# thuml/iVideoGPT

Hardware: AMD Instinct MI355X
Metric: predicted frames/sec (encode+GPT rollout+decode), 64x64x16f (higher is better)
Workload: dtype bf16; 1 GPU; ivideogpt-oxe-64-act-free (BASELINE config 2): synthetic 64x64 bf16 clips, 64 trajectories per GPU, 2 context + 14 predicted frames, top-k 100 sampling, seeded random weights; global_batch=64, frames=16, resolution=64, lanes=4

## Files before the change

include/ivg.h:

```cpp
#ifndef IVG_H_
#define IVG_H_

#include <stddef.h>
#include <stdint.h>

#ifdef __cplusplus
extern "C" {
#endif

typedef struct ivg_engine ivg_engine;
typedef struct ivg_cache ivg_cache;
typedef void* ivg_stream;

enum ivg_dtype { IVG_F32 = 0, IVG_BF16 = 1, IVG_F32X3 = 2 };

enum ivg_status {
  IVG_OK = 0,
  IVG_ERR_INVALID = -1,
  IVG_ERR_MISSING = -2,
  IVG_ERR_HIP = -3,
  IVG_ERR_CAPACITY = -4
};

typedef struct {
// ... 92 lines not shown
                        void* hidden_out, int allow_reuse, int* reused_out, ivg_stream stream);
int ivg_reward_linear(ivg_engine* e, const void* hidden, int rows, float* out, ivg_stream stream);

int ivg_logits(ivg_engine* e, const int64_t* ids, int B, int L, const float* actions, int act_T, int ctx, float* logits_out,
               ivg_stream stream);

int ivg_eval_forward(ivg_engine* e, const int64_t* ids, const int64_t* labels, int B, int L, const float* actions, int act_T, int ctx,
                     float* token_nll_out, float* loss_rows_out, void* hidden_out, ivg_stream stream);
int ivg_action_recon_sqerr(ivg_engine* e, const void* hidden, const float* actions, int B, int L, int act_T, int ctx, int prelude, float* out,
                           ivg_stream stream);

int ivg_ingest_frames(const uint8_t* frames, int T, int H, int W, int center_crop, void* clip_out, int out_dtype, int resolution,
                      ivg_stream stream);

size_t ivg_frame_metrics_ws_bytes(int n_samples, int T, int H, int W);
int ivg_frame_metrics(const void* gt, int gt_dtype, int B, int T_gt, int gt_t0, const float* pred, int n_samples, int T_pr, int pr_t0, int T, int H,
                      int W, float* rows_out, void* ws, size_t ws_bytes, ivg_stream stream);

typedef struct ivg_lpips ivg_lpips;
int ivg_lpips_create(const ivg_tensor* weights, int n_weights, int device, ivg_lpips** out);
void ivg_lpips_destroy(ivg_lpips* p);
size_t ivg_lpips_ws_bytes(int max_images_per_chunk, int H, int W);
int ivg_lpips_rows(ivg_lpips* p, const void* gt, int gt_dtype, int B, int T_gt, int gt_t0, const float* pred, int n_samples, int T_pr, int pr_t0, int T,
                   int H, int W, float* frames_out, float* rows_out, void* ws, size_t ws_bytes, ivg_stream stream);

enum ivg_kernel_class { IVG_K_IGEMM_BF16 = 0, IVG_K_IGEMM_F32 = 1, IVG_K_CONV3X3_BF16 = 2, IVG_K_CONV3X3_F32 = 3, IVG_K_DECODE_ATTN = 4,
                        IVG_K_DECODE_GEMM = 5,
                        IVG_K_COUNT = 6 };
typedef struct {
  int64_t launches;
  double total_ms;
  double total_flops;
  double total_bytes;
} ivg_profile_stats;
int ivg_profile_enable(ivg_engine* e, int kernel_class, int enable);
int ivg_profile_read(ivg_engine* e, int kernel_class, ivg_profile_stats* out);
int ivg_profile_attn_fit(ivg_engine* e, double* fixed_us, double* gbps);
int ivg_profile_gemm_kinds(ivg_engine* e, double* mean_us, int64_t* launches);

typedef struct {
  const void* X; const void* W; void* Y; const void* R; const float* bias;
  int32_t Nimg, Hin, Win, Cin, ldx, Hout, Wout, KH, KW, stride, pad, ups, N, ldw;
  int64_t c_img, c_pix, c_ch, c_grp_stride;
  int32_t c_grp, flags;
  float alpha;
  int32_t nb0, nb1, nb2;
  int64_t sa[3], sw[3], sy[3];
} ivg_igemm_args;
int ivg_op_igemm(const ivg_igemm_args* a, int dtype, ivg_stream stream);
int ivg_op_conv_gn(const ivg_igemm_args* a, int dtype, void* gn_part, int groups, const float* gamma, const float* beta, void* gn_out, float eps,
                   int silu, ivg_stream stream);
int ivg_op_gn_conv(const ivg_igemm_args* a, int dtype, int groups, const float* gamma, const float* beta, float eps, void* ws, ivg_stream stream);
int ivg_op_conv_x3(const ivg_igemm_args* a, const void* w_x3, int groups, const float* gamma, const float* beta, float eps, void* ws,
                   ivg_stream stream);
int ivg_op_conv_subpixel(const ivg_igemm_args* a, int dtype, const void* w_sub, const void* w_x3, const void* w_sub_x3, void* gn_part, int groups,
                         ivg_stream stream);
int ivg_op_conv3x3(const ivg_igemm_args* a, int dtype, const float* gamma, const float* beta, int in_groups, float eps, void* ws,
                   const void* in_part, int in_chunks, void* gn_part, int groups, const void* w_x3, const void* w_sub, const void* w_sub_x3,
                   ivg_stream stream);
#define IVG_CONV3X3_PLAN_INTS 15
int ivg_op_conv3x3_plan(const ivg_igemm_args* a, int dtype, int gn_in, int gn_groups, const void* w_x3, const void* w_sub,
                        const void* w_sub_x3, int32_t* out);
int ivg_op_xattn(const void* q, const void* Kp, const void* VpT, void* out, int M, int F, int P, int kv, int C, int nh, int dtype, ivg_stream stream);
int ivg_op_skinny(const void* X, const void* W, void* Y, int M, int N, int K, int ldx, int ldw, int ldy, int flags, int dtype,
                  ivg_stream stream);
int ivg_op_skinny_policy(const void* X, const void* W, void* Y, int M, int N, int K, int ldx, int ldw, int ldy, int flags, int dtype, int lds_kb,
                         int w_shared, ivg_stream stream);
#define IVG_SKINNY_PLAN_INTS 11
int ivg_op_skinny_plan(int M, int N, int K, int ldx, int ldw, int ldy, int flags, int dtype, int lds_kb, const void* X, const void* W,
                       const void* Y, int32_t* out);
int ivg_op_groupnorm(const void* X, void* Y, void* ws , const float* gamma, const float* beta,
                     const float* pos, int N, int P, int C, int groups, float eps, int silu, int dtype, ivg_stream stream);
int ivg_op_softmax(const float* S, void* P, int64_t rows, int Lq, int Lk, int lds, int ldp, int causal, int dtype,
                   ivg_stream stream);
int ivg_op_vq_argmin(const float* z, const float* codebook, float* ee_ws , int64_t* out, int R, int n_e,
                     ivg_stream stream);
int ivg_op_add_rmsnorm(void* x, const float* w, void* out, int M, int H, float eps, int dtype, ivg_stream stream);
int ivg_op_conv_in(const void* video, int video_dtype, const float* w, const float* bias, void* Y, int dtype, int N, int per,
                   int T_total, int t0, int H, int W, int C0, ivg_stream stream);
int ivg_op_shared_decode_attn(const void* qkv, void* kc, void* vc, void* out, const float* cos_t, const float* sin_t, int B, int heads, int hd, int Lmax,
                              int pos, int P, int G, int row0, int dtype, ivg_stream stream);
int ivg_op_prefill_attn(void* qkv, void* kc, void* vc, void* vt, void* out, const float* cos_t, const float* sin_t, int B, int L, int heads, int hd,
                        int Lmax, int dtype, ivg_stream stream);
int ivg_op_kv24_pack(const float* k32, const float* v32, void* kc, void* vc, int BH, int L, int Lmax, ivg_stream stream);
int ivg_op_decode_attn24(const float* qkv, void* kc, void* vc, float* out, const float* cos_t, const float* sin_t, int B, int heads, int Lmax, int pos,
                         int P, int G, int row0, ivg_stream stream);
int ivg_op_kv8_pack(const void* k16, const void* v16, void* kc, void* vc, int BH, int L, int Lmax, float k_scale, float v_scale, ivg_stream stream);
int ivg_op_decode_attn8(const void* qkv, void* kc, void* vc, void* out, const float* cos_t, const float* sin_t, int B, int heads, int Lmax, int pos,
                        int P, int G, int row0, float k_scale, float v_scale, ivg_stream stream);
int ivg_op_kv8_pack_heads(const void* k16, const void* v16, void* kc, void* vc, int B, int heads, int L, int Lmax, const float* k_scales,
                          const float* v_scales, ivg_stream stream);
int ivg_op_decode_attn8_heads(const void* qkv, void* kc, void* vc, void* out, const float* cos_t, const float* sin_t, int B, int heads, int Lmax, int pos,
                              int P, int G, int row0, const float* k_scales, const float* v_scales, ivg_stream stream);
int ivg_op_kv_absmax(const void* k16, const void* v16, int B, int heads, int L, int Lmax, uint32_t* out, ivg_stream stream);
int ivg_op_sample(const float* logits, int B, int V, int top_k, float temperature, const float* uniforms, int64_t* out, ivg_stream stream);
int ivg_op_sample_top_p(const float* logits, int B, int V, int top_k, float temperature, float top_p, const float* uniforms, int64_t* out,
                        ivg_stream stream);
int ivg_op_lpips_features(ivg_lpips* p, const void* images, int dtype, int n, int H, int W, float* const* taps_out, void* ws, size_t ws_bytes,
                          ivg_stream stream);
int ivg_op_lpips_head(const float* f0, const float* f1, const float* lin, int n0, int n1, int P, int C, float* out, void* ws, size_t ws_bytes,
                      ivg_stream stream);
int ivg_op_lpips_conv_in(const void* images, int dtype, const float* w, const float* bias, float* Y, int n, int H, int W, ivg_stream stream);
int ivg_op_maxpool2(const float* X, float* Y, int N, int H, int W, int C, ivg_stream stream);
int64_t ivg_debug_counter(const char* name);

#ifdef __cplusplus
}
#endif
#endif
```

ivideogpt_amd/_lib.py:

```python
import ctypes as C
import os

_HERE = os.path.dirname(os.path.abspath(__file__))
LIB_PATH = os.path.join(_HERE, "lib", "libivg.so")

IVG_F32, IVG_BF16, IVG_F32X3 = 0, 1, 2
IVG_K_IGEMM_BF16, IVG_K_IGEMM_F32, IVG_K_CONV3X3_BF16, IVG_K_CONV3X3_F32, IVG_K_DECODE_ATTN, IVG_K_DECODE_GEMM = 0, 1, 2, 3, 4, 5
IG_BIAS_N, IG_BIAS_M, IG_RESIDUAL, IG_SILU, IG_GLU, IG_OUT_F32 = 1, 2, 4, 8, 16, 32
IG_RELU = 256
IVG_KV_NATIVE, IVG_KV_FP8_E4M3 = 0, 1


class IvgTensor(C.Structure):
    _fields_ = [("name", C.c_char_p), ("data", C.c_void_p), ("dtype", C.c_int32), ("ndim", C.c_int32),
                ("shape", C.c_int64 * 4)]


class IvgConfig(C.Structure):
    _fields_ = [
        ("n_levels", C.c_int32), ("block_out_channels", C.c_int32 * 8), ("layers_per_block", C.c_int32),
        ("latent_channels", C.c_int32), ("vq_embed_dim", C.c_int32), ("num_vq_embeddings", C.c_int32),
        ("num_dyn_embeddings", C.c_int32), ("norm_num_groups", C.c_int32), ("mid_block_add_attention", C.c_int32),
        ("context_length", C.c_int32), ("max_att_resolution", C.c_int32), ("resolution", C.c_int32),
        ("patch_size", C.c_int32),
# ... 30 lines not shown
    "ivg_create": (C.c_int, [C.POINTER(IvgConfig), C.POINTER(IvgTensor), C.c_int, C.c_int, C.POINTER(C.c_void_p)]),
    "ivg_destroy": (None, [C.c_void_p]),
    "ivg_reload_switches": (None, []),
    "ivg_set_temperature": (C.c_int, [C.c_void_p, C.c_float]),
    "ivg_set_top_p": (C.c_int, [C.c_void_p, C.c_float]),
    "ivg_set_decode_lds_kb": (C.c_int, [C.c_void_p, C.c_int]),
    "ivg_set_kv_format": (C.c_int, [C.c_void_p, C.c_int, C.c_float, C.c_float]),
    "ivg_set_kv_scales": (C.c_int, [C.c_void_p, C.c_void_p]),
    "ivg_get_kv_scales": (C.c_int, [C.c_void_p, C.c_void_p]),
    "ivg_kv_calibrate": (C.c_int, [C.c_void_p, C.c_void_p, C.c_int64, C.c_int, C.c_int, C.c_void_p, C.c_int, C.c_int, C.c_void_p]),
    "ivg_kv_calibration_reset": (C.c_int, [C.c_void_p]),
    "ivg_kv_calibration_finish": (C.c_int, [C.c_void_p, C.c_int, C.c_void_p, C.c_void_p]),
    "ivg_set_context_length": (C.c_int, [C.c_void_p, C.c_int]),
    "ivg_tokenize": (C.c_int, [C.c_void_p, C.c_void_p, C.c_int, C.c_int, C.c_int, C.c_void_p, C.c_void_p, C.c_void_p]),
    "ivg_encode_context": (C.c_int, [C.c_void_p, C.c_void_p, C.c_int, C.c_int, C.c_int, C.c_void_p, C.c_int64, C.c_void_p]),
    "ivg_detokenize": (C.c_int, [C.c_void_p, C.c_void_p, C.c_int, C.c_int, C.c_void_p, C.c_void_p, C.c_int, C.c_void_p]),
    "ivg_detokenize_shared": (C.c_int, [C.c_void_p, C.c_void_p, C.c_int, C.c_int, C.c_int, C.c_void_p, C.c_int, C.c_void_p]),
    "ivg_detokenize_to": (C.c_int, [C.c_void_p, C.c_void_p, C.c_int, C.c_int, C.c_void_p, C.c_int, C.c_void_p, C.c_int, C.c_void_p]),
    "ivg_set_output_clamp": (C.c_int, [C.c_void_p, C.c_int]),
    "ivg_cache_create": (C.c_int, [C.c_void_p, C.c_int, C.POINTER(C.c_void_p)]),
    "ivg_cache_destroy": (None, [C.c_void_p, C.c_void_p]),
    "ivg_generate": (C.c_int, [C.c_void_p, C.c_void_p, C.c_int64, C.c_int, C.c_int, C.c_int, C.c_void_p, C.c_int, C.c_int,
                               C.c_void_p, C.c_int, C.c_void_p, C.c_void_p, C.c_void_p]),
    "ivg_generate_shared": (C.c_int, [C.c_void_p, C.c_void_p, C.c_int64, C.c_int, C.c_int, C.c_int, C.c_int, C.c_void_p, C.c_int, C.c_int,
                                      C.c_void_p, C.c_int, C.c_int, C.c_void_p, C.c_void_p, C.c_void_p]),
    "ivg_generate_forced_sdf": (C.c_int, [C.c_void_p, C.c_void_p, C.c_int64, C.c_int, C.c_int, C.c_int, C.c_int, C.c_void_p, C.c_int, C.c_void_p,
                                         C.c_void_p]),
    "ivg_generate_continue": (C.c_int, [C.c_void_p, C.c_void_p, C.c_int64, C.c_int, C.c_int, C.c_int, C.c_void_p, C.c_int, C.c_int,
                                        C.c_void_p, C.c_int, C.c_void_p, C.c_void_p, C.c_void_p]),
    "ivg_embed_tokens": (C.c_int, [C.c_void_p, C.c_void_p, C.c_int64, C.c_int, C.c_int, C.c_void_p, C.c_void_p]),
    "ivg_action_linear": (C.c_int, [C.c_void_p, C.c_void_p, C.c_int, C.c_void_p, C.c_void_p]),
    "ivg_generate_embeds": (C.c_int, [C.c_void_p, C.c_void_p, C.c_int, C.c_int, C.c_int, C.c_void_p, C.c_int, C.c_void_p, C.c_void_p,
                                      C.c_int, C.POINTER(C.c_int), C.c_void_p]),
    "ivg_reward_linear": (C.c_int, [C.c_void_p, C.c_void_p, C.c_int, C.c_void_p, C.c_void_p]),
    "ivg_logits": (C.c_int, [C.c_void_p, C.c_void_p, C.c_int, C.c_int, C.c_void_p, C.c_int, C.c_int, C.c_void_p, C.c_void_p]),
    "ivg_eval_forward": (C.c_int, [C.c_void_p, C.c_void_p, C.c_void_p, C.c_int, C.c_int, C.c_void_p, C.c_int, C.c_int, C.c_void_p,
                                   C.c_void_p, C.c_void_p, C.c_void_p]),
    "ivg_action_recon_sqerr": (C.c_int, [C.c_void_p, C.c_void_p, C.c_void_p, C.c_int, C.c_int, C.c_int, C.c_int, C.c_int, C.c_void_p,
                                         C.c_void_p]),
    "ivg_ingest_frames": (C.c_int, [C.c_void_p, C.c_int, C.c_int, C.c_int, C.c_int, C.c_void_p, C.c_int, C.c_int, C.c_void_p]),
    "ivg_frame_metrics_ws_bytes": (C.c_size_t, [C.c_int, C.c_int, C.c_int, C.c_int]),
    "ivg_frame_metrics": (C.c_int, [C.c_void_p, C.c_int, C.c_int, C.c_int, C.c_int, C.c_void_p, C.c_int, C.c_int, C.c_int, C.c_int, C.c_int,
                                    C.c_int, C.c_void_p, C.c_void_p, C.c_size_t, C.c_void_p]),
    "ivg_lpips_create": (C.c_int, [C.POINTER(IvgTensor), C.c_int, C.c_int, C.POINTER(C.c_void_p)]),
    "ivg_lpips_destroy": (None, [C.c_void_p]),
    "ivg_lpips_ws_bytes": (C.c_size_t, [C.c_int, C.c_int, C.c_int]),
    "ivg_lpips_rows": (C.c_int, [C.c_void_p, C.c_void_p] + [C.c_int] * 4 + [C.c_void_p] + [C.c_int] * 6 + [C.c_void_p] * 3 + [C.c_size_t, C.c_void_p]),
    "ivg_op_lpips_features": (C.c_int, [C.c_void_p, C.c_void_p] + [C.c_int] * 4 + [C.POINTER(C.c_void_p), C.c_void_p, C.c_size_t, C.c_void_p]),
    "ivg_op_lpips_head": (C.c_int, [C.c_void_p] * 3 + [C.c_int] * 4 + [C.c_void_p, C.c_void_p, C.c_size_t, C.c_void_p]),
    "ivg_op_lpips_conv_in": (C.c_int, [C.c_void_p, C.c_int, C.c_void_p, C.c_void_p, C.c_void_p] + [C.c_int] * 3 + [C.c_void_p]),
    "ivg_op_maxpool2": (C.c_int, [C.c_void_p, C.c_void_p] + [C.c_int] * 4 + [C.c_void_p]),
    "ivg_profile_enable": (C.c_int, [C.c_void_p, C.c_int, C.c_int]),
    "ivg_profile_read": (C.c_int, [C.c_void_p, C.c_int, C.POINTER(IvgProfileStats)]),
    "ivg_profile_attn_fit": (C.c_int, [C.c_void_p, C.POINTER(C.c_double), C.POINTER(C.c_double)]),
    "ivg_profile_gemm_kinds": (C.c_int, [C.c_void_p, C.POINTER(C.c_double), C.POINTER(C.c_int64)]),
    "ivg_op_igemm": (C.c_int, [C.POINTER(IvgIgemmArgs), C.c_int, C.c_void_p]),
    "ivg_op_conv_gn": (C.c_int, [C.POINTER(IvgIgemmArgs), C.c_int, C.c_void_p, C.c_int, C.c_void_p, C.c_void_p, C.c_void_p, C.c_float, C.c_int,
                                 C.c_void_p]),
    "ivg_op_gn_conv": (C.c_int, [C.POINTER(IvgIgemmArgs), C.c_int, C.c_int, C.c_void_p, C.c_void_p, C.c_float, C.c_void_p, C.c_void_p]),
    "ivg_op_conv_x3": (C.c_int, [C.POINTER(IvgIgemmArgs), C.c_void_p, C.c_int, C.c_void_p, C.c_void_p, C.c_float, C.c_void_p, C.c_void_p]),
    "ivg_op_conv3x3": (C.c_int, [C.POINTER(IvgIgemmArgs), C.c_int, C.c_void_p, C.c_void_p, C.c_int, C.c_float, C.c_void_p, C.c_void_p, C.c_int,
                                 C.c_void_p, C.c_int, C.c_void_p, C.c_void_p, C.c_void_p, C.c_void_p]),
    "ivg_op_conv3x3_plan": (C.c_int, [C.POINTER(IvgIgemmArgs), C.c_int, C.c_int, C.c_int, C.c_void_p, C.c_void_p, C.c_void_p,
                                      C.POINTER(C.c_int32)]),
    "ivg_op_xattn": (C.c_int, [C.c_void_p] * 4 + [C.c_int] * 7 + [C.c_void_p]),
    "ivg_op_conv_subpixel": (C.c_int, [C.c_void_p, C.c_int, C.c_void_p, C.c_void_p, C.c_void_p, C.c_void_p, C.c_int, C.c_void_p]),
    "ivg_op_shared_decode_attn": (C.c_int, [C.c_void_p] * 6 + [C.c_int] * 9 + [C.c_void_p]),
    "ivg_op_prefill_attn": (C.c_int, [C.c_void_p] * 7 + [C.c_int] * 6 + [C.c_void_p]),
    "ivg_op_kv24_pack": (C.c_int, [C.c_void_p] * 4 + [C.c_int] * 3 + [C.c_void_p]),
    "ivg_op_decode_attn24": (C.c_int, [C.c_void_p] * 6 + [C.c_int] * 7 + [C.c_void_p]),
    "ivg_op_kv8_pack": (C.c_int, [C.c_void_p] * 4 + [C.c_int] * 3 + [C.c_float, C.c_float, C.c_void_p]),
    "ivg_op_decode_attn8": (C.c_int, [C.c_void_p] * 6 + [C.c_int] * 7 + [C.c_float, C.c_float, C.c_void_p]),
    "ivg_op_kv8_pack_heads": (C.c_int, [C.c_void_p] * 4 + [C.c_int] * 4 + [C.c_void_p] * 3),
    "ivg_op_decode_attn8_heads": (C.c_int, [C.c_void_p] * 6 + [C.c_int] * 7 + [C.c_void_p] * 3),
    "ivg_op_kv_absmax": (C.c_int, [C.c_void_p] * 2 + [C.c_int] * 4 + [C.c_void_p] * 2),
    "ivg_op_skinny": (C.c_int, [C.c_void_p, C.c_void_p, C.c_void_p] + [C.c_int] * 8 + [C.c_void_p]),
    "ivg_op_skinny_policy": (C.c_int, [C.c_void_p, C.c_void_p, C.c_void_p] + [C.c_int] * 10 + [C.c_void_p]),
    "ivg_op_skinny_plan": (C.c_int, [C.c_int] * 9 + [C.c_void_p] * 3 + [C.POINTER(C.c_int32)]),
    "ivg_op_groupnorm": (C.c_int, [C.c_void_p] * 6 + [C.c_int] * 4 + [C.c_float, C.c_int, C.c_int, C.c_void_p]),
    "ivg_op_softmax": (C.c_int, [C.c_void_p, C.c_void_p, C.c_int64] + [C.c_int] * 6 + [C.c_void_p]),
    "ivg_op_vq_argmin": (C.c_int, [C.c_void_p] * 4 + [C.c_int, C.c_int, C.c_void_p]),
    "ivg_op_add_rmsnorm": (C.c_int, [C.c_void_p, C.c_void_p, C.c_void_p, C.c_int, C.c_int, C.c_float, C.c_int, C.c_void_p]),
    "ivg_op_conv_in": (C.c_int, [C.c_void_p, C.c_int, C.c_void_p, C.c_void_p, C.c_void_p] + [C.c_int] * 8 + [C.c_void_p]),
    "ivg_op_sample": (C.c_int, [C.c_void_p, C.c_int, C.c_int, C.c_int, C.c_float, C.c_void_p, C.c_void_p, C.c_void_p]),
    "ivg_op_sample_top_p": (C.c_int, [C.c_void_p, C.c_int, C.c_int, C.c_int, C.c_float, C.c_float, C.c_void_p, C.c_void_p, C.c_void_p]),
    "ivg_debug_counter": (C.c_int64, [C.c_char_p]),
}

_lib = None


def load():
    global _lib
    if _lib is not None:
        return _lib
    if not os.path.exists(LIB_PATH):
        raise RuntimeError(
            f"{LIB_PATH} is missing: the HIP engine has not been built (make -C ivideogpt_amd/csrc). "
            "ivideogpt_amd has no CPU / PyTorch fallback path.")
    lib = C.CDLL(LIB_PATH)
    for name, (res, args) in EXPORTS.items():
        fn = getattr(lib, name)
        fn.restype, fn.argtypes = res, args
    _lib = lib
    return lib


def reload_switches():
    load().ivg_reload_switches()


def last_error(handle=None):
    msg = load().ivg_last_error(handle)
    return msg.decode() if msg else ""


class IvgError(RuntimeError):
    pass


def check(rc, handle=None, what=""):
    if rc != 0:
        msg = f"{what}: libivg error {rc}: {last_error(handle)}"
        if rc == -1:
            raise AssertionError(msg)
        raise IvgError(msg)
```

ivideogpt_amd/csrc/api.cpp:

```cpp
#include <cstdlib>
#include <cstring>

#include <cstdio>
#include "engine_impl.h"
#include "switches.h"

using namespace ivg;

static thread_local std::string g_create_err;

namespace ivg {

size_t dtype_size(DType d) { return d == BF16 ? 2 : 4; }

struct Lookup {
  ivg_engine* e;
  bool ok = true;
  const ivg_tensor* find(const std::string& name, int dtype, int64_t numel) {
    auto it = e->wmap.find(name);
    if (it == e->wmap.end()) { if (ok) e->err = "missing weight tensor '" + name + "'"; ok = false; return nullptr; }
    const ivg_tensor& t = it->second;
    int64_t n = 1;
    for (int i = 0; i < t.ndim; ++i) n *= t.shape[i];
    if (t.dtype != dtype || n != numel) {
// ... 585 lines not shown
                        ivg_stream stream) {
  if (!e) return IVG_ERR_INVALID;
  const bool sized = n_groups > 0 && group_size > 0;
  const int B = sized ? n_groups * group_size : 1;
  IVG_TRY(check_generate(e, GEN_SHARED, sized ? nullptr : "generate_shared: n_groups and group_size must be positive", B, L0, n_new, actions, act_T, ctx));
  GenerateReq q; q.prompt = prompts; q.prompt_stride = prompt_stride; q.B = B; q.L0 = L0; q.n_new = n_new; q.actions = actions; q.act_T = act_T; q.ctx = ctx;
  q.uniforms = uniforms; q.top_k = top_k; q.ids_out = ids_out; q.reward_out = reward_out; q.force_sdf = force_sdf != 0;
  q.group = group_size;
  return plan_then_run(e, (hipStream_t)stream, [&](Run& r) { return r.generate(q); });
}

int ivg_generate_forced_sdf(ivg_engine* e, const int64_t* prompt, int64_t prompt_stride, int B, int L0, int n_new, int ctx, const float* uniforms,
                            int top_k, int64_t* ids_out, ivg_stream stream) {
  if (!e) return IVG_ERR_INVALID;
  IVG_TRY(check_generate(e, GEN_PLAIN, nullptr, B, L0, n_new, nullptr, 0, ctx));
  GenerateReq q; q.prompt = prompt; q.prompt_stride = prompt_stride; q.B = B; q.L0 = L0; q.n_new = n_new; q.ctx = ctx;
  q.uniforms = uniforms; q.top_k = top_k; q.ids_out = ids_out; q.force_sdf = true;
  return plan_then_run(e, (hipStream_t)stream, [&](Run& r) { return r.generate(q); });
}

int ivg_generate_continue(ivg_engine* e, const int64_t* prompt, int64_t prompt_stride, int B, int L0, int n_new, const float* actions,
                          int act_T, int ctx, const float* uniforms, int top_k, int64_t* ids_out, float* reward_out, ivg_stream stream) {
  if (!e) return IVG_ERR_INVALID;
  const bool act_ok = actions && e->cfg.action_dim > 0 && e->act_w;
  IVG_TRY(check_generate(e, GEN_CONTINUE, act_ok ? nullptr : "generate_continue: action-conditioned models only", B, L0, n_new, actions, act_T, ctx));
  if (!e->kvc.holds(B, L0 - 1))
    return e->fail(IVG_ERR_INVALID, "generate_continue: the KV cache holds " + std::to_string(e->kvc.len) + " positions of " + std::to_string(e->kvc.B) +
                                        " trajectories, the call needs " + std::to_string(L0 - 1) + " of " + std::to_string(B));
  {
    bool same = false;
    IVG_TRY(kv_prefix_matches_ids(e, prompt, prompt_stride, B, L0, actions, act_T, ctx, (hipStream_t)stream, &same));
    if (!same) return e->fail(IVG_ERR_INVALID, "generate_continue: the KV cache was built from a different prefix (tokens or actions differ)");
  }
  GenerateReq q; q.prompt = prompt; q.prompt_stride = prompt_stride; q.B = B; q.L0 = L0; q.n_new = n_new; q.actions = actions; q.act_T = act_T; q.ctx = ctx;
  q.uniforms = uniforms; q.top_k = top_k; q.ids_out = ids_out; q.reward_out = reward_out; q.reuse_kv = true;
  return plan_then_run(e, (hipStream_t)stream, [&](Run& r) { return r.generate(q); });
}

int ivg_generate_embeds(ivg_engine* e, const void* embeds, int B, int L0, int n_new, const float* uniforms, int top_k, int64_t* new_ids_out,
                        void* hidden_out, int allow_reuse, int* reused_out, ivg_stream stream) {
  if (!e) return IVG_ERR_INVALID;
  if (reused_out) *reused_out = 0;
  IVG_TRY(check_generate(e, GEN_EMBEDS, embeds && new_ids_out ? nullptr : "generate_embeds: null argument", B, L0, n_new, nullptr, 0, 1));
  bool reuse = false;
  if (allow_reuse && L0 >= 2) IVG_TRY(kv_prefix_matches_embeds(e, embeds, B, L0, (hipStream_t)stream, &reuse));
  if (reused_out) *reused_out = reuse ? 1 : 0;
  GenerateReq q; q.B = B; q.L0 = L0; q.n_new = n_new; q.uniforms = uniforms; q.top_k = top_k;
  q.reuse_kv = reuse; q.embeds = embeds; q.new_ids_out = new_ids_out; q.hidden_out = hidden_out;
  return plan_then_run(e, (hipStream_t)stream, [&](Run& r) { return r.generate(q); });
}

int ivg_embed_tokens(ivg_engine* e, const int64_t* ids, int64_t ids_stride, int B, int L, void* out, ivg_stream stream) {
  if (!e) return IVG_ERR_INVALID;
  if (e->cfg.num_layers <= 0 || !e->embed) return e->fail(IVG_ERR_INVALID, "embed_tokens: engine was created without a transformer");
  if (B <= 0 || L <= 0) return IVG_OK;
  if (launch_embed(ids, ids_stride, e->embed, out, e->llm_dt, B, L, e->cfg.hidden_size, e->cfg.vocab_size, (hipStream_t)stream))
    return e->fail(IVG_ERR_HIP, "embed_tokens: launch failed");
  return IVG_OK;
}

int ivg_action_linear(ivg_engine* e, const float* actions, int rows, void* out, ivg_stream stream) {
  if (!e) return IVG_ERR_INVALID;
  if (e->cfg.action_dim <= 0 || !e->act_w) return e->fail(IVG_ERR_INVALID, "action_linear: the model is action-free");
  if (launch_action_embed(actions, e->act_w, e->act_b, out, e->llm_dt, rows, e->cfg.action_dim, e->cfg.hidden_size, (hipStream_t)stream))
    return e->fail(IVG_ERR_HIP, "action_linear: launch failed");
  return IVG_OK;
}

int ivg_reward_linear(ivg_engine* e, const void* hidden, int rows, float* out, ivg_stream stream) {
  if (!e) return IVG_ERR_INVALID;
  if (!e->rew_w_raw || !e->rew_b) return e->fail(IVG_ERR_MISSING, "reward_linear: the model has no reward head");
  if (launch_rowdot(hidden, e->rew_w_raw, e->rew_b, out, rows, e->cfg.hidden_size, -1.0f, e->llm_dt, (hipStream_t)stream))
    return e->fail(IVG_ERR_HIP, "reward_linear: launch failed");
  return IVG_OK;
}

int ivg_logits(ivg_engine* e, const int64_t* ids, int B, int L, const float* actions, int act_T, int ctx, float* logits_out, ivg_stream stream) {
  if (!e) return IVG_ERR_INVALID;
  if (e->cfg.num_layers <= 0) return e->fail(IVG_ERR_INVALID, "logits: engine was created without a transformer");
  if (B <= 0 || B > e->kvc.chunk || L > e->Lmax) return e->fail(IVG_ERR_CAPACITY, "logits: batch or length exceeds capacity");
  if (actions && (e->cfg.action_dim <= 0 || !e->act_w)) return e->fail(IVG_ERR_INVALID, "logits: actions given but the model is action-free");
  return plan_then_run(e, (hipStream_t)stream, [&](Run& r) {
    PrefillReq q; q.ids = ids; q.ids_stride = L; q.B = B; q.L = L; q.act_T = act_T; q.ctx = ctx; q.all_slots = true; q.logits_all = logits_out;
    IVG_TRY(embed_actions(r, actions, B * act_T, &q.act_emb));
    return r.prefill(q);
  });
}

int ivg_eval_forward(ivg_engine* e, const int64_t* ids, const int64_t* labels, int B, int L, const float* actions, int act_T, int ctx,
                     float* token_nll_out, float* loss_rows_out, void* hidden_out, ivg_stream stream) {
  if (!e) return IVG_ERR_INVALID;
  if (e->cfg.num_layers <= 0) return e->fail(IVG_ERR_INVALID, "eval_forward: engine was created without a transformer");
  if (!ids || !labels || !token_nll_out || !loss_rows_out) return e->fail(IVG_ERR_INVALID, "eval_forward: null argument");
  if (B <= 0 || B > e->kvc.chunk || L < 2 || L > e->Lmax) return e->fail(IVG_ERR_CAPACITY, "eval_forward: batch or length exceeds capacity");
  if (actions && (e->cfg.action_dim <= 0 || !e->act_w)) return e->fail(IVG_ERR_INVALID, "eval_forward: actions given but the model is action-free");
  return plan_then_run(e, (hipStream_t)stream, [&](Run& r) {
    PrefillReq q; q.ids = ids; q.ids_stride = L; q.B = B; q.L = L; q.act_T = act_T; q.ctx = ctx; q.all_slots = true;
    q.hidden_all = hidden_out; q.labels = labels; q.token_nll = token_nll_out;
    IVG_TRY(embed_actions(r, actions, B * act_T, &q.act_emb));
    IVG_TRY(r.prefill(q));
    if (!r.planning && launch_ce_reduce(token_nll_out, labels, B, L, e->cfg.vocab_size, loss_rows_out, r.st)) return e->fail(IVG_ERR_HIP, "ce_reduce launch failed");
    return 0;
  });
}

int ivg_action_recon_sqerr(ivg_engine* e, const void* hidden, const float* actions, int B, int L, int act_T, int ctx, int prelude, float* out,
                           ivg_stream stream) {
  if (!e) return IVG_ERR_INVALID;
  if (!e->ar_w || !e->ar_b) return e->fail(IVG_ERR_MISSING, "action_recon: 'action_recon_linear' is not in the weight table");
  if (!hidden || !actions || !out || B <= 0 || prelude < 0 || prelude >= L) return e->fail(IVG_ERR_INVALID, "action_recon: bad argument");
  if (ctx - 1 + (L - 1 - prelude) / 17 >= act_T) return e->fail(IVG_ERR_INVALID, "action_recon: action tensor too short");
  if (launch_action_recon(hidden, e->ar_w, e->ar_b, actions, B, L, e->cfg.hidden_size, e->cfg.action_dim, act_T, ctx, prelude, out, e->llm_dt,
                          (hipStream_t)stream))
    return e->fail(IVG_ERR_HIP, "action_recon: launch failed");
  return IVG_OK;
}

int ivg_ingest_frames(const uint8_t* frames, int T, int H, int W, int center_crop, void* clip_out, int out_dtype, int resolution, ivg_stream stream) {
  if (!frames || !clip_out || (out_dtype != IVG_F32 && out_dtype != IVG_BF16)) return IVG_ERR_INVALID;
  const int rc = launch_ingest(frames, T, H, W, center_crop, clip_out, (DType)out_dtype, resolution, (hipStream_t)stream);
  return rc == 0 ? IVG_OK : (rc == (int)hipErrorInvalidValue ? IVG_ERR_INVALID : IVG_ERR_HIP);
}

size_t ivg_frame_metrics_ws_bytes(int n_samples, int T, int H, int W) { return frame_metrics_ws_bytes(n_samples, T, H, W); }

int ivg_frame_metrics(const void* gt, int gt_dtype, int B, int T_gt, int gt_t0, const float* pred, int n_samples, int T_pr, int pr_t0, int T, int H,
                      int W, float* rows_out, void* ws, size_t ws_bytes, ivg_stream stream) {
  if (!gt || !pred || !rows_out || !ws) return IVG_ERR_INVALID;
  if (B <= 0 || n_samples <= 0 || n_samples % B != 0 || T <= 0 || gt_t0 < 0 || pr_t0 < 0 || gt_t0 + T > T_gt || pr_t0 + T > T_pr || H < 11 || W < 11)
    return IVG_ERR_INVALID;
  if (ws_bytes < frame_metrics_ws_bytes(n_samples, T, H, W)) return IVG_ERR_CAPACITY;
  return launch_frame_metrics(gt, (DType)gt_dtype, B, T_gt, gt_t0, pred, n_samples, T_pr, pr_t0, T, H, W, rows_out, ws, (hipStream_t)stream) ? IVG_ERR_HIP
                                                                                                                                                : IVG_OK;
}

struct ivg_lpips {
  int device = 0;
  const float* cw[13];
  const float* cb[13];
  const float* lin[5];
};

int ivg_lpips_create(const ivg_tensor* weights, int n_weights, int device, ivg_lpips** out) {
  if (!out) return IVG_ERR_INVALID;
  *out = nullptr;
  if (!weights || n_weights <= 0) { g_create_err = "no weight table"; return IVG_ERR_MISSING; }
  static const int idx[13] = {0, 2, 5, 7, 10, 12, 14, 17, 19, 21, 24, 26, 28}, slice[13] = {1, 1, 2, 2, 3, 3, 3, 4, 4, 4, 5, 5, 5};
  static const int cin[13] = {3, 64, 64, 128, 128, 256, 256, 256, 512, 512, 512, 512, 512}, cout[13] = {64, 64, 128, 128, 256, 256, 256, 512, 512, 512, 512, 512, 512};
  static const int tapc[5] = {64, 128, 256, 512, 512};
  int status = IVG_OK;
  auto find = [&](const std::string& name, int64_t numel) -> const float* {
    for (int i = 0; i < n_weights; ++i) {
      if (!weights[i].name || name != weights[i].name) continue;
      int64_t n = 1;
      for (int d = 0; d < weights[i].ndim; ++d) n *= weights[i].shape[d];
      if (weights[i].dtype != IVG_F32 || n != numel || !weights[i].data || ((uintptr_t)weights[i].data & 15)) {
        if (status == IVG_OK) { status = IVG_ERR_INVALID; g_create_err = "LPIPS weight tensor '" + name + "': expected " + std::to_string(numel) + " float32 elements, 16-byte aligned"; }
        return nullptr;
      }
      return (const float*)weights[i].data;
    }
    if (status == IVG_OK) { status = IVG_ERR_MISSING; g_create_err = "missing LPIPS weight tensor '" + name + "'"; }
    return nullptr;
  };
  ivg_lpips h;
  h.device = device;
// ... 222 lines not shown
  g.gn_in_coef = coef;
  const int rc = launch_conv3x3(g, (DType)dtype, (hipStream_t)stream);
  return rc == 0 ? IVG_OK : (rc > 0 ? IVG_ERR_HIP : IVG_ERR_INVALID);
}

int ivg_op_conv_x3(const ivg_igemm_args* a, const void* w_x3, int groups, const float* gamma, const float* beta, float eps, void* ws, ivg_stream stream) {
  IgemmArgs g;
  igemm_op_args(g, a);
  g.W_x3 = w_x3;
  if (!w_x3) return IVG_ERR_INVALID;
  if (gamma) {
    const int P = a->Hin * a->Win, nch = gn_num_chunks(P);
    char* part = (char*)ws;
    char* coef = part + (size_t)a->Nimg * nch * groups * 16;
    if (launch_groupnorm_partial(a->X, part, a->Nimg, P, a->Cin, groups, F32, (hipStream_t)stream)) return IVG_ERR_HIP;
    if (launch_gn_coef(part, nch, gamma, beta, a->Nimg, P, a->Cin, groups, eps, coef, (hipStream_t)stream)) return IVG_ERR_HIP;
    g.gn_in_coef = coef;
  }
  const int rc = launch_conv3x3(g, F32, (hipStream_t)stream);
  return rc == 0 ? IVG_OK : (rc > 0 ? IVG_ERR_HIP : IVG_ERR_INVALID);
}

static bool conv3x3_op_args(IgemmArgs& g, DType& dt, const ivg_igemm_args* a, int dtype, const void* w_x3, const void* w_sub, const void* w_sub_x3) {
  if (!a || (dtype != IVG_F32 && dtype != IVG_BF16 && dtype != IVG_F32X3)) return false;
  if (dtype == IVG_F32X3 && !w_x3) return false;
  igemm_op_args(g, a);
  g.nb0 = a->nb0; g.nb1 = a->nb1; g.nb2 = a->nb2;
  g.W_x3 = w_x3; g.W_sub = w_sub; g.W_sub_x3 = w_sub_x3;
  dt = dtype == IVG_BF16 ? BF16 : F32;
  return true;
}

int ivg_op_conv3x3(const ivg_igemm_args* a, int dtype, const float* gamma, const float* beta, int in_groups, float eps, void* ws,
                   const void* in_part, int in_chunks, void* gn_part, int groups, const void* w_x3, const void* w_sub, const void* w_sub_x3,
                   ivg_stream stream) {
  IgemmArgs g;
  DType dt;
  if (!conv3x3_op_args(g, dt, a, dtype, w_x3, w_sub, w_sub_x3)) return IVG_ERR_INVALID;
  g.gn_part = gn_part; g.gn_groups = groups;
  char* coef = nullptr;
  const int P = a->Hin * a->Win;
  if (gamma) {
    if (!beta || !ws || in_groups <= 0 || a->Cin % in_groups != 0 || P <= 0 || a->Nimg <= 0 || (in_part && in_chunks <= 0)) return IVG_ERR_INVALID;
    coef = (char*)ws + (size_t)a->Nimg * gn_num_chunks(P) * in_groups * 16;
    g.gn_in_coef = coef;
  }
  if (conv3x3_plan(g, dt).covered != 1) return IVG_ERR_INVALID;
  if (gamma) {
    const void* part = in_part;
    int nch = in_chunks;
    if (!part) {
      if (launch_groupnorm_partial(a->X, ws, a->Nimg, P, a->Cin, in_groups, dt, (hipStream_t)stream)) return IVG_ERR_HIP;
      part = ws; nch = gn_num_chunks(P);
    }
    if (launch_gn_coef(part, nch, gamma, beta, a->Nimg, P, a->Cin, in_groups, eps, coef, (hipStream_t)stream)) return IVG_ERR_HIP;
  }
  const int rc = launch_conv3x3(g, dt, (hipStream_t)stream);
  if (rc != 0) return rc > 0 ? IVG_ERR_HIP : IVG_ERR_INVALID;
  return g.gn_chunks;
}

int ivg_op_conv3x3_plan(const ivg_igemm_args* a, int dtype, int gn_in, int gn_groups, const void* w_x3, const void* w_sub,
                        const void* w_sub_x3, int32_t* out) {
  IgemmArgs g;
  DType dt;
  if (!out || !conv3x3_op_args(g, dt, a, dtype, w_x3, w_sub, w_sub_x3)) return IVG_ERR_INVALID;
  if (gn_in) g.gn_in_coef = (const void*)out;
  if (gn_groups > 0) { g.gn_part = (void*)out; g.gn_groups = gn_groups; }
  const Conv3Plan p = conv3x3_plan(g, dt);
  const int32_t v[IVG_CONV3X3_PLAN_INTS] = {p.covered, p.kind, p.bn, p.tw, p.ups, p.gna, p.tpb2, p.subpix, p.tiles_x, p.tiles_per_img, p.tiles_n,
                                            p.chunks, p.staged, p.gn_chunks, p.lds_bytes};
  for (int i = 0; i < IVG_CONV3X3_PLAN_INTS; ++i) out[i] = v[i];
  return IVG_OK;
}

int64_t ivg_debug_counter(const char* name) {
  if (name && !strcmp(name, "conv3x3_subpixel")) return conv3x3_subpixel_launches();
  if (name && !strcmp(name, "gemm256x3")) return gemm256x3_launches();
  if (name && !strcmp(name, "decode_attn24")) return decode_attn24_launches();
  if (name && !strcmp(name, "decode_attn8")) return decode_attn8_launches();
  if (name && !strcmp(name, "decode_gemm_gen3")) return decode_gemm_launches(3);
  if (name && !strcmp(name, "decode_gemm_gen2")) return decode_gemm_launches(2);
  if (name && !strcmp(name, "lpips_trunk_images")) return lpips_trunk_images();
  return -1;
}

int ivg_op_skinny(const void* X, const void* W, void* Y, int M, int N, int K, int ldx, int ldw, int ldy, int flags, int dtype, ivg_stream stream) {
  return ivg_op_skinny_policy(X, W, Y, M, N, K, ldx, ldw, ldy, flags, dtype, 0, 0, stream);
}

static bool skinny_op_args(SkinnyArgs& s, DType& dt, int M, int N, int K, int ldx, int ldw, int ldy, int flags, int dtype, int lds_kb) {
  if (dtype != IVG_F32 && dtype != IVG_BF16 && dtype != IVG_F32X3) return false;
  if (lds_kb != 0 && (lds_kb < 16 || lds_kb > 160)) return false;
  s.M = M; s.N = N; s.K = K; s.ldx = ldx; s.ldw = ldw; s.ldy = ldy; s.flags = flags; s.lds_kb = lds_kb;
  s.x3 = dtype == IVG_F32X3;
  dt = dtype == IVG_BF16 ? BF16 : F32;
  return true;
}

int ivg_op_skinny_policy(const void* X, const void* W, void* Y, int M, int N, int K, int ldx, int ldw, int ldy, int flags, int dtype, int lds_kb,
                         int w_shared, ivg_stream stream) {
  SkinnyArgs s;
  DType dt;
  if (!skinny_op_args(s, dt, M, N, K, ldx, ldw, ldy, flags, dtype, lds_kb)) return IVG_ERR_INVALID;
  s.X = X; s.W = W; s.Y = Y; s.w_shared = w_shared != 0;
  return launch_skinny(s, dt, (hipStream_t)stream) ? IVG_ERR_HIP : IVG_OK;
}

int ivg_op_skinny_plan(int M, int N, int K, int ldx, int ldw, int ldy, int flags, int dtype, int lds_kb, const void* X, const void* W,
                       const void* Y, int32_t* out) {
  SkinnyArgs s;
  DType dt;
  if (!out || !skinny_op_args(s, dt, M, N, K, ldx, ldw, ldy, flags, dtype, lds_kb)) return IVG_ERR_INVALID;
  s.X = X; s.W = W; s.Y = (void*)Y;
  const SkinnyPlan p = skinny_plan(s, dt);
  const int32_t v[IVG_SKINNY_PLAN_INTS] = {p.gen, p.mf, p.fn, p.waves, p.klw, p.ring, p.lg, p.nburst, p.wmax, p.wr, p.x3};
  for (int i = 0; i < IVG_SKINNY_PLAN_INTS; ++i) out[i] = v[i];
  return IVG_OK;
}

int ivg_op_groupnorm(const void* X, void* Y, void* ws, const float* gamma, const float* beta, const float* pos, int N, int P, int C, int groups,
                     float eps, int silu, int dtype, ivg_stream stream) {
  return launch_groupnorm(X, Y, ws, gamma, beta, pos, N, P, C, groups, eps, silu, (DType)dtype, (hipStream_t)stream) ? IVG_ERR_HIP : IVG_OK;
}

int ivg_op_softmax(const float* S, void* P, int64_t rows, int Lq, int Lk, int lds, int ldp, int causal, int dtype, ivg_stream stream) {
  return launch_softmax(S, P, rows, Lq, Lk, lds, ldp, causal, (DType)dtype, (hipStream_t)stream) ? IVG_ERR_HIP : IVG_OK;
}

int ivg_op_vq_argmin(const float* z, const float* codebook, float* ee_ws, int64_t* out, int R, int n_e, ivg_stream stream) {
  if (launch_sqnorm_rows(codebook, ee_ws, n_e, 64, (hipStream_t)stream)) return IVG_ERR_HIP;
  TokMap mp{1, 1, 1, 0, 1};
  return launch_vq_argmin(z, codebook, ee_ws, out, mp, 0, R, n_e, (hipStream_t)stream) ? IVG_ERR_HIP : IVG_OK;
}

int ivg_op_add_rmsnorm(void* x, const float* w, void* out, int M, int H, float eps, int dtype, ivg_stream stream) {
  return launch_add_rmsnorm(x, H, w, out, M, H, eps, (DType)dtype, (hipStream_t)stream) ? IVG_ERR_HIP : IVG_OK;
}

int ivg_op_conv_in(const void* video, int video_dtype, const float* w, const float* bias, void* Y, int dtype, int N, int per, int T_total, int t0,
                   int H, int W, int C0, ivg_stream stream) {
  return launch_conv_in(video, (DType)video_dtype, w, bias, Y, (DType)dtype, N, per, T_total, t0, H, W, C0, (hipStream_t)stream) ? IVG_ERR_HIP : IVG_OK;
}

int ivg_op_shared_decode_attn(const void* qkv, void* kc, void* vc, void* out, const float* cos_t, const float* sin_t, int B, int heads, int hd, int Lmax,
                              int pos, int P, int G, int row0, int dtype, ivg_stream stream) {
  if (B <= 0 || heads <= 0 || G < 1 || P < 0 || P > pos || pos >= Lmax || row0 > 0) return IVG_ERR_INVALID;
  if ((dtype != IVG_F32 && dtype != IVG_BF16) || !decode_attn_covers(hd, (DType)dtype)) return IVG_ERR_INVALID;
  return one_step(pos, stream, [&](StepState* state, hipStream_t st) {
    return launch_decode_attn(qkv, kc, vc, out, cos_t, sin_t, B, heads, hd, Lmax, state, nullptr, (DType)dtype, st, P, G, row0); });
}

int ivg_op_prefill_attn(void* qkv, void* kc, void* vc, void* vt, void* out, const float* cos_t, const float* sin_t, int B, int L, int heads,
                        int hd, int Lmax, int dtype, ivg_stream stream) {
  if (B <= 0 || heads <= 0 || L < 1 || L > Lmax || hd <= 0 || hd % 2 || (dtype != IVG_F32 && dtype != IVG_BF16)) return IVG_ERR_INVALID;
  if (out && (dtype != IVG_BF16 || hd != 64 || !vt || ((uintptr_t)qkv & 15) || ((uintptr_t)out & 7))) return IVG_ERR_INVALID;
  const int Lp = (L + 63) / 64 * 64;
  hipStream_t st = (hipStream_t)stream;
  int rc = launch_rope_kv(qkv, kc, vc, vt, Lp, cos_t, sin_t, B, L, heads, hd, Lmax, nullptr, 0, (DType)dtype, st);
  if (rc == 0 && out) rc = launch_flash_prefill(qkv, kc, vt, out, B, L, Lp, heads, hd, Lmax, (DType)dtype, st);
  return rc == 0 ? IVG_OK : (rc > 0 ? IVG_ERR_HIP : IVG_ERR_INVALID);
}

int ivg_op_kv24_pack(const float* k32, const float* v32, void* kc, void* vc, int BH, int L, int Lmax, ivg_stream stream) {
  if (BH <= 0 || L < 0 || L > Lmax) return IVG_ERR_INVALID;
  return launch_kv24_pack(k32, v32, kc, vc, BH, L, Lmax, (hipStream_t)stream) ? IVG_ERR_HIP : IVG_OK;
// ... 71 lines not shown
```

ivideogpt_amd/csrc/common.h:

```cpp
#pragma once
#include <hip/hip_runtime.h>
#include <stdint.h>

#include <atomic>
#include <mutex>

namespace ivg {

typedef __bf16 bf16_t;
typedef bf16_t bf16x8 __attribute__((ext_vector_type(8)));
typedef bf16_t bf16x4 __attribute__((ext_vector_type(4)));
typedef bf16_t bf16x2 __attribute__((ext_vector_type(2)));
typedef float f32x4 __attribute__((ext_vector_type(4)));
typedef float f32x2 __attribute__((ext_vector_type(2)));

enum DType : int { F32 = 0, BF16 = 1 };

typedef uint32_t Chunk16 __attribute__((ext_vector_type(4)));

template <typename T> struct Traits;
template <> struct Traits<float> {
  static constexpr int VEC = 4;
  static constexpr DType dtype = F32;
};
template <> struct Traits<bf16_t> {
  static constexpr int VEC = 8;
  static constexpr DType dtype = BF16;
};

__device__ __forceinline__ float to_f32(float v) { return v; }
__device__ __forceinline__ float to_f32(bf16_t v) { return (float)v; }
template <typename T> __device__ __forceinline__ T from_f32(float v);
template <> __device__ __forceinline__ float from_f32<float>(float v) { return v; }
template <> __device__ __forceinline__ bf16_t from_f32<bf16_t>(float v) { return (bf16_t)v; }

__device__ __forceinline__ float silu_f(float v) { return v / (1.0f + __expf(-v)); }
template <typename T> __device__ __forceinline__ float silu_t(float v) {
  if constexpr (sizeof(T) == 2) return v * __builtin_amdgcn_rcpf(1.0f + __expf(-v));
  else return silu_f(v);
}

__device__ __forceinline__ float wave_sum(float v) {
#pragma unroll
  for (int o = 32; o > 0; o >>= 1) v += __shfl_xor(v, o, 64);
  return v;
}
__device__ __forceinline__ double wave_sum(double v) {
#pragma unroll
  for (int o = 32; o > 0; o >>= 1) v += __shfl_xor(v, o, 64);
  return v;
}
__device__ __forceinline__ float wave_max(float v) {
#pragma unroll
  for (int o = 32; o > 0; o >>= 1) v = fmaxf(v, __shfl_xor(v, o, 64));
  return v;
}

template <int CTRL> __device__ __forceinline__ float dpp_add_f32(float v) {
  return v + __int_as_float(__builtin_amdgcn_update_dpp(0, __float_as_int(v), CTRL, 0xf, 0xf, false));
}
__device__ __forceinline__ float row16_sum(float d) {
  d = dpp_add_f32<0xB1>(d);
  d = dpp_add_f32<0x4E>(d);
  d = dpp_add_f32<0x141>(d);
  d = dpp_add_f32<0x140>(d);
  return d;
}

static inline int cdiv(long a, long b) { return (int)((a + b - 1) / b); }

struct DynLdsOnce { std::atomic<unsigned long long> done{0}; std::mutex mu; };
static inline hipError_t ensure_dyn_lds(DynLdsOnce& g, const void* fn, int bytes) {
  int d = 0;
  (void)hipGetDevice(&d);
  const unsigned long long bit = 1ull << (d & 63);
  if (g.done.load(std::memory_order_acquire) & bit) return hipSuccess;
  std::lock_guard<std::mutex> lk(g.mu);
  if (g.done.load(std::memory_order_relaxed) & bit) return hipSuccess;
  const hipError_t e = hipFuncSetAttribute(fn, hipFuncAttributeMaxDynamicSharedMemorySize, bytes);
  if (e == hipSuccess) g.done.fetch_or(bit, std::memory_order_release);
  return e;
}

}
```

ivideogpt_amd/csrc/conv_small.hip:

```cpp
#include "ops.h"

namespace ivg {

template <typename TI, typename TO>
__global__ __launch_bounds__(256) void conv_in_kernel(const TI* __restrict__ video, const float* __restrict__ w,
                                                      const float* __restrict__ bias, TO* __restrict__ Y, int N, int per,
                                                      int T_total, int t0, int H, int W, int C0) {
  extern __shared__ __attribute__((aligned(16))) unsigned char smem[];
  float* sw = (float*)smem;
  float* sb = sw + 27 * C0;
  for (int i = threadIdx.x; i < 27 * C0; i += 256) {
    const int co = i / 27, k = i - co * 27;
    sw[k * C0 + co] = w[i];
  }
  for (int i = threadIdx.x; i < C0; i += 256) sb[i] = bias[i];
  __syncthreads();
  const int cgn = C0 / 8;
  const long total = (long)N * H * W * cgn;
  for (long idx = (long)blockIdx.x * 256 + threadIdx.x; idx < total; idx += (long)gridDim.x * 256) {
    const int cg = (int)(idx % cgn);
    long t = idx / cgn;
    const int ow = (int)(t % W); t /= W;
    const int oh = (int)(t % H);
    const int n = (int)(t / H);
    const long fr = (long)(n / per) * T_total + t0 + (n % per);
    const TI* src = video + fr * 3 * H * W;
    float acc[8];
#pragma unroll
    for (int j = 0; j < 8; ++j) acc[j] = sb[cg * 8 + j];
#pragma unroll
    for (int ci = 0; ci < 3; ++ci)
#pragma unroll
      for (int kh = 0; kh < 3; ++kh)
#pragma unroll
        for (int kw = 0; kw < 3; ++kw) {
          const int ih = oh + kh - 1, iw = ow + kw - 1;
          float x = 0.f;
          if (ih >= 0 && ih < H && iw >= 0 && iw < W) x = to_f32(src[((long)ci * H + ih) * W + iw]);
          const float* wk = sw + (ci * 9 + kh * 3 + kw) * C0 + cg * 8;
#pragma unroll
          for (int j = 0; j < 8; ++j) acc[j] = fmaf(x, wk[j], acc[j]);
        }
    TO* o = Y + (((long)n * H + oh) * W + ow) * C0 + cg * 8;
    if constexpr (sizeof(TO) == 2) {
      bf16x8 v;
#pragma unroll
      for (int j = 0; j < 8; ++j) v[j] = (bf16_t)acc[j];
      *(bf16x8*)o = v;
    } else {
      *(f32x4*)o = f32x4{acc[0], acc[1], acc[2], acc[3]};
      *(f32x4*)(o + 4) = f32x4{acc[4], acc[5], acc[6], acc[7]};
    }
  }
}

int launch_conv_in(const void* video, DType video_dt, const float* w, const float* bias, void* Y, DType dt, int N, int per,
                   int T_total, int t0, int H, int W, int C0, hipStream_t st) {
  if (C0 % 8 != 0 || N <= 0) return N <= 0 ? 0 : (int)hipErrorInvalidValue;
  const long total = (long)N * H * W * (C0 / 8);
  const int blocks = (int)(total / 256 > 16384 ? 16384 : cdiv(total, 256));
  const size_t smem = (size_t)(28 * C0) * sizeof(float);
  dim3 g(blocks), b(256);
#define IVG_CI(TI, TO) hipLaunchKernelGGL((conv_in_kernel<TI, TO>), g, b, smem, st, (const TI*)video, w, bias, (TO*)Y, N, per, T_total, t0, H, W, C0)
  if (video_dt == F32 && dt == F32) IVG_CI(float, float);
  else if (video_dt == F32 && dt == BF16) IVG_CI(float, bf16_t);
  else if (video_dt == BF16 && dt == F32) IVG_CI(bf16_t, float);
  else IVG_CI(bf16_t, bf16_t);
#undef IVG_CI
  return (int)hipGetLastError();
}

}
```

ivideogpt_amd/csrc/engine_impl.h:

```cpp
#pragma once
#include <algorithm>
#include <cmath>
#include <string>
#include <vector>

#include "engine.h"

namespace ivg {

#define IVG_TRY(x) do { int _r = (x); if (_r != 0) return _r; } while (0)

struct GnStats { void* part = nullptr; int chunks = 0; };

struct PrefillReq {
  const int64_t* ids = nullptr; int64_t ids_stride = 0; int B = 0, L = 0;
  const void* act_emb = nullptr; int act_T = 0, ctx = 1; bool all_slots = false;
  float* logits_all = nullptr;
  float* logits_last = nullptr; void* hidden_last = nullptr;
  const void* embeds = nullptr;
  void* hidden_all = nullptr;
  const int64_t* labels = nullptr; float* token_nll = nullptr;
};

struct GenerateReq {
  const int64_t* prompt = nullptr; int64_t prompt_stride = 0; int B = 0, L0 = 0, n_new = 0;
  const float* actions = nullptr; int act_T = 0, ctx = 1;
  const float* uniforms = nullptr; int top_k = 0;
  int64_t* ids_out = nullptr; float* reward_out = nullptr;
  bool reuse_kv = false;
  const void* embeds = nullptr; int64_t* new_ids_out = nullptr; void* hidden_out = nullptr;
  bool force_sdf = false;
  int group = 1;
};

struct Run {
  ivg_engine* e;
  hipStream_t st;
  bool planning;
  bool x3 = false;
  unsigned int* kv_amax = nullptr;
  int kv_group = 1;

  int conv(DType dt, const void* X, int N, int H, int W, const ConvW& c, void* Y, int stride, int ups, const void* Rres, int flags,
           int out_f32, GnStats* out_stats = nullptr ,
           const void* in_coef = nullptr );
  int norm_conv(DType dt, const void* x, int N, int H, int W, const NormW& n, float eps, const GnStats* x_stats, const ConvW& c, void* Y,
                const void* Rres, void* scratch, GnStats* out_stats);
  int gemm(DType dt, const IgemmArgs& a, double flops, double bytes);
  int linear(DType dt, const void* X, long rows, const ConvW& c, void* Y, const void* Rres, int flags, int out_f32);
  int gnorm(DType dt, const void* X, void* Y, int N, int P, int C, const NormW& n, float eps, int silu, const float* pos,
            const GnStats* stats = nullptr );
  int resnet(DType dt, const void* x, int N, int H, int W, const ResnetW& r, void* out, const GnStats* x_stats = nullptr,
             GnStats* out_stats = nullptr);
  size_t gn_stats_bytes(int N, int H, int W, int C) const;
  int self_attention(DType dt, const void* x, int N, int P, int C, const AttnW& a, void* out);
  int xatt_project_kv(DType dt, const void* feat, int B, const XAttW& x, void* Kp, void* VpT);
  int cross_attention(DType dt, const void* z, int B, int F, const XAttW& x, const void* Kp, const void* VpT, void* out);
  int encoder_trunk(const TrunkW& w, const void* pixels, DType pix_dt, int B, int per, int T_total, int t0,
                    std::vector<Feature>* keep, const std::vector<Feature>* cond, void* latent);
  int decoder_trunk(const TrunkW& w, const void* z, int B, int per, int T_total, int t0, std::vector<Feature>* keep,
                    const std::vector<Feature>* cond, void* out_pixels, DType out_dt);
  int tokenize(const void* pixels, DType pix_dt, int B, int T, int64_t* ids, int64_t ids_stride, int64_t* labels, bool ctx_only);
  int detokenize(const int64_t* ids, int B, int F, void* out_pixels, DType out_dt, ivg_cache* cache, int cache_mode,
                 int group = 1 );

  int prefill(const PrefillReq& q);
  int generate(const GenerateReq& q);

  void prof_begin(DType dt, double flops, double bytes, int base = 0);
  void prof_end(DType dt, int base = 0);
  void prof_cancel(DType dt, int base = 0);
};

size_t dtype_size(DType d);
int build_tokenizer(ivg_engine* e);
int build_transformer(ivg_engine* e);
size_t gen_buffer_bytes(const ivg_engine* e);
int kv_prefix_matches_ids(ivg_engine* e, const int64_t* prompt, int64_t prompt_stride, int B, int L0, const float* actions, int act_T,
                          int ctx, hipStream_t st, bool* ok);
int kv_prefix_matches_embeds(ivg_engine* e, const void* embeds, int B, int L0, hipStream_t st, bool* ok);

}
```

ivideogpt_amd/csrc/gemm256.hip:

```cpp
#include <algorithm>
#include <atomic>
#include <cstdlib>

#include "igemm.h"
#include "switches.h"

namespace ivg {

struct G256Dev {
  const bf16_t* X; const bf16_t* W; bf16_t* Y; const bf16_t* R; const float* bias;
  int M, N, K, ldx, ldw, ldy;
  int tiles_n;
  int flags;
  int tiles_m, gn;
};

template <typename Dev>
__device__ __forceinline__ void g256_tile(const Dev& p, int v, int& tile_m, int& tile_n) {
  const int per_group = p.gn * p.tiles_m;
  const int g = v / per_group, rem = v - g * per_group;
  const int gsize = min(p.gn, p.tiles_n - g * p.gn);
  tile_m = rem / gsize;
  tile_n = g * p.gn + (rem - tile_m * gsize);
}
// ... 197 lines not shown
  __builtin_amdgcn_s_barrier();
  for (int s = 0; s < steps; ++s) {
    if (s + 1 < steps) issue(s + 1);
    const unsigned char* sa = smem + (s & 1) * G256L_STAGE;
    const unsigned char* sw_ = sa + G256L_HALF;
#pragma unroll
    for (int tt = 0; tt < 2; ++tt) {
      const int slot = fslot0 + ((tt * 4 + lg) ^ fkey);
      Chunk16 xs[4];
#pragma unroll
      for (int b = 0; b < 4; ++b) xs[b] = g256_split_hi_lo(*(const Chunk16*)(sa + ((wm * 4 + b) * 128 + slot) * 16));
#pragma unroll
      for (int a = 0; a < 4; ++a) {
        const Chunk16 ws = g256_split_hi_lo(*(const Chunk16*)(sw_ + ((wn * 4 + a) * 128 + slot) * 16));
#pragma unroll
        for (int h = 0; h < 2; ++h) {
          Chunk16 wd = Chunk16{ws[2 * h], ws[2 * h + 1], ws[2 * h], ws[2 * h + 1]};
          asm volatile("" : "+v"(wd));
#pragma unroll
          for (int b0 = 0; b0 < 4; ++b0) {
            const int b = ((a * 2 + h) & 1) ? 3 - b0 : b0;
            acc[a][b] = __builtin_amdgcn_mfma_f32_16x16x32_bf16(__builtin_bit_cast(bf16x8, wd), __builtin_bit_cast(bf16x8, xs[b]),
                                                                acc[a][b], 0, 0, 0);
          }
        }
      }
    }
    asm volatile("s_waitcnt vmcnt(0) lgkmcnt(0)" ::: "memory");
    __builtin_amdgcn_s_barrier();
  }
  const int flags = p.flags;
  const bool glu = flags & IG_GLU;
  const int out_n0 = glu ? (n0 >> 1) : n0;
#pragma unroll
  for (int b = 0; b < 4; ++b) {
    const int m = m0 + wm * 64 + b * 16 + lr;
    if (m >= p.M) continue;
#pragma unroll
    for (int a = 0; a < 4; ++a) {
      if (glu && (a & 1)) continue;
      float v4[4];
#pragma unroll
      for (int r = 0; r < 4; ++r) v4[r] = acc[a][b][r];
      const int ncol = wn * 64 + a * 16 + lg * 4;
      if (flags & IG_BIAS_N) {
#pragma unroll
        for (int r = 0; r < 4; ++r) v4[r] += p.bias[n0 + ncol + r];
      }
      int ocol = ncol;
      if (glu) {
        const int a1 = a + 1 < 4 ? a + 1 : a;
#pragma unroll
        for (int r = 0; r < 4; ++r) v4[r] = silu_t<float>(v4[r]) * acc[a1][b][r];
        ocol = (wn * 64 + a * 16) / 2 + lg * 4;
      }
      float* dst = p.Y + (long)m * p.ldy + out_n0 + ocol;
      if (flags & IG_RESIDUAL) {
        const f32x4 rv = *(const f32x4*)(p.R + (long)m * p.ldy + out_n0 + ocol);
#pragma unroll
        for (int r = 0; r < 4; ++r) v4[r] += rv[r];
      }
      if (flags & IG_SILU) {
#pragma unroll
        for (int r = 0; r < 4; ++r) v4[r] = silu_t<float>(v4[r]);
      }
      *(f32x4*)dst = f32x4{v4[0], v4[1], v4[2], v4[3]};
    }
  }
}

static std::atomic<long long> g_gemm256x3_launches{0};
long long gemm256x3_launches() { return g_gemm256x3_launches.load(); }

static int launch_gemm256_x3(const IgemmArgs& a, hipStream_t stream) {
  if (!sw().gemm256) return -1;
  if (a.KH != 1 || a.KW != 1 || a.stride != 1 || a.pad != 0 || a.ups) return -1;
  if (a.nb0 * a.nb1 * a.nb2 != 1 || a.alpha != 1.0f) return -1;
  if (a.flags & ~(IG_BIAS_N | IG_RESIDUAL | IG_SILU | IG_GLU | IG_OUT_F32)) return -1;
  const long M = (long)a.Nimg * a.Hout * a.Wout;
  if (a.Hout != a.Hin || a.Wout != a.Win || a.ldx != a.Cin) return -1;
  if (a.c_ch != 1 || (a.c_grp > 1)) return -1;
  if (a.Nimg > 1 && a.c_img != (long)a.Hout * a.Wout * a.c_pix) return -1;
  const bool glu = a.flags & IG_GLU;
  if (M < 4096 || a.N % 256 != 0 || a.Cin % 32 != 0 || a.Cin < 64 || a.ldw % 4 != 0 || a.c_pix % 4 != 0) return -1;
  if (((uintptr_t)a.X & 15) || ((uintptr_t)a.W & 15) || ((uintptr_t)a.Y & 15) || ((a.flags & IG_RESIDUAL) && ((uintptr_t)a.R & 15))) return -1;
  if (glu && (a.flags & IG_BIAS_N)) return -1;
  if ((long)a.N * a.ldw * 4 >= (1L << 32)) return -1;
  const long row_bytes = 4L * std::max<long>(a.ldx, a.c_pix);
  const long rows_max = ((1L << 32) - 1) / row_bytes / 256 * 256;
  if (rows_max < 4096) return -1;
  static DynLdsOnce once_x;
  for (long r0 = 0; r0 < M; r0 += rows_max) {
    const long rows = std::min(rows_max, M - r0);
    G256XDev d;
    d.X = (const float*)a.X + r0 * a.ldx; d.W = (const float*)a.W; d.Y = (float*)a.Y + r0 * a.c_pix;
    d.R = a.R ? (const float*)a.R + r0 * a.c_pix : nullptr; d.bias = a.bias;
    d.M = (int)rows; d.N = a.N; d.K = a.Cin; d.ldx = a.ldx; d.ldw = a.ldw; d.ldy = (int)a.c_pix;
    d.tiles_n = a.N / 256;
    d.flags = a.flags;
    d.tiles_m = cdiv(rows, 256);
    {
      const long slab = 256L * d.K * 4;
      d.gn = (int)std::max(1L, std::min<long>((5L << 19) / slab, d.tiles_n));
    }
    const long tiles = (long)cdiv(rows, 256) * d.tiles_n;
    if (hipError_t e = ensure_dyn_lds(once_x, (const void*)gemm256x3_kernel, 160 * 1024); e != hipSuccess) return (int)e;
    hipLaunchKernelGGL(gemm256x3_kernel, dim3((unsigned)tiles), dim3(1024), 2 * G256L_STAGE, stream, d);
    if (hipError_t e = hipGetLastError(); e != hipSuccess) return (int)e;
    g_gemm256x3_launches.fetch_add(1);
  }
  return 0;
}

int launch_gemm256(const IgemmArgs& a, DType dtype, hipStream_t stream) {
  if (dtype == F32 && a.x3 && sw().gemm256x3) return launch_gemm256_x3(a, stream);
  if (dtype != BF16 || !sw().gemm256) return -1;
  if (a.KH != 1 || a.KW != 1 || a.stride != 1 || a.pad != 0 || a.ups) return -1;
  if (a.nb0 * a.nb1 * a.nb2 != 1 || a.alpha != 1.0f) return -1;
  if (a.flags & ~(IG_BIAS_N | IG_RESIDUAL | IG_SILU | IG_GLU)) return -1;
  const long M = (long)a.Nimg * a.Hout * a.Wout;
  if (a.Hout != a.Hin || a.Wout != a.Win || a.ldx != a.Cin) return -1;
  if (a.c_ch != 1 || (a.c_grp > 1)) return -1;
  if (a.Nimg > 1 && a.c_img != (long)a.Hout * a.Wout * a.c_pix) return -1;
  const bool glu = a.flags & IG_GLU;
  const int BN = a.N % 256 == 0 ? 256 : 128;
  if (BN == 128 && (glu || M < (1L << 18))) return -1;
  if (M < 4096 || M > 0x7fffffffL || a.N % 128 != 0 || a.Cin % 32 != 0 || a.Cin < 64 || a.ldw % 8 != 0 || a.c_pix % 8 != 0) return -1;
  if (((uintptr_t)a.X & 15) || ((uintptr_t)a.W & 15) || ((uintptr_t)a.Y & 15) || ((a.flags & IG_RESIDUAL) && ((uintptr_t)a.R & 7))) return -1;
  if (glu && (a.flags & IG_BIAS_N)) return -1;
  if (a.Cin % 64 != 0 || (long)a.N * a.ldw * 2 >= (1L << 31)) return -1;
  const long row_bytes = 2L * std::max<long>(a.ldx, a.c_pix);
  long rows_max = ((1L << 31) - 1) / row_bytes / 256 * 256;
  if (rows_max < 4096) return -1;
  static DynLdsOnce once_l, once_h;
  const int smem_l = 256 * G256_PITCH > 2 * G256L_STAGE ? 256 * G256_PITCH : 2 * G256L_STAGE;
  for (long r0 = 0; r0 < M; r0 += rows_max) {
    const long rows = std::min(rows_max, M - r0);
    G256Dev d;
    d.X = (const bf16_t*)a.X + r0 * a.ldx; d.W = (const bf16_t*)a.W; d.Y = (bf16_t*)a.Y + r0 * a.c_pix;
    d.R = a.R ? (const bf16_t*)a.R + r0 * a.c_pix : nullptr; d.bias = a.bias;
    d.M = (int)rows; d.N = a.N; d.K = a.Cin; d.ldx = a.ldx; d.ldw = a.ldw; d.ldy = (int)a.c_pix;
    d.tiles_n = a.N / BN;
    d.flags = a.flags;
    d.tiles_m = cdiv(rows, 256);
    {
      const long slab = (long)BN * d.K * 2;
      d.gn = (int)std::max(1L, std::min<long>((5L << 19) / slab, d.tiles_n));
    }
    const long tiles = (long)cdiv(rows, 256) * d.tiles_n;
    if (BN == 256) {
      if (hipError_t e = ensure_dyn_lds(once_l, (const void*)gemm256l_kernel<256>, 160 * 1024); e != hipSuccess) return (int)e;
      hipLaunchKernelGGL(gemm256l_kernel<256>, dim3((unsigned)tiles), dim3(1024), smem_l, stream, d);
    } else {
      if (hipError_t e = ensure_dyn_lds(once_h, (const void*)gemm256l_kernel<128>, 160 * 1024); e != hipSuccess) return (int)e;
      hipLaunchKernelGGL(gemm256l_kernel<128>, dim3((unsigned)tiles), dim3(1024), smem_l, stream, d);
    }
    if (hipError_t e = hipGetLastError(); e != hipSuccess) return (int)e;
  }
  return 0;
}

}
```

ivideogpt_amd/csrc/igemm.h:

```cpp
#pragma once
#include "common.h"

namespace ivg {

enum IgemmFlags : int {
  IG_BIAS_N = 1,
  IG_BIAS_M = 2,
  IG_RESIDUAL = 4,
  IG_SILU = 8,
  IG_GLU = 16,
  IG_OUT_F32 = 32,
  SK_NORM = 64,
  IG_CLAMP01 = 128,
  IG_RELU = 256,
};

struct IgemmArgs {
  const void* X = nullptr;
  const void* W = nullptr;
  void* Y = nullptr;
  const void* R = nullptr;
  const float* bias = nullptr;
  int Nimg = 1, Hin = 1, Win = 1, Cin = 0, ldx = 0;
  int Hout = 1, Wout = 1;
  int KH = 1, KW = 1, stride = 1, pad = 0, ups = 0;
  int N = 0, ldw = 0;
  long c_img = 0, c_pix = 0, c_ch = 1;
  int c_grp = 1;
  long c_grp_stride = 0;
  int flags = 0;
  float alpha = 1.0f;
  void* gn_part = nullptr;
  int gn_groups = 0;
  mutable int gn_chunks = 0;
  const void* gn_in_coef = nullptr;
  const void* W_x3 = nullptr;
  const void* W_sub = nullptr;
  const void* W_sub_x3 = nullptr;
  bool x3 = false;
  int nb0 = 1, nb1 = 1, nb2 = 1;
  long sa[3] = {0, 0, 0}, sw[3] = {0, 0, 0}, sy[3] = {0, 0, 0};
};

int launch_igemm(const IgemmArgs& a, DType dtype, hipStream_t stream);
int launch_gemm256(const IgemmArgs& a, DType dtype, hipStream_t stream);
int launch_conv3x3(const IgemmArgs& a, DType dtype, hipStream_t stream);
struct Conv3Plan {
  int covered = 0, kind = 0, bn = 0, tw = 0, ups = 0, gna = 0, tpb2 = 0, subpix = 0;
  int tiles_x = 0, tiles_per_img = 0, tiles_n = 0, chunks = 0, staged = 0, gn_chunks = 0, lds_bytes = 0;
  int stage_ok = 0, gn_off = 0, coef_off = 0;
};
Conv3Plan conv3x3_plan(const IgemmArgs& a, DType dtype);
long long gemm256x3_launches();
long long conv3x3_subpixel_launches();
long long decode_gemm_launches(int generation);
int conv3x3_gn_chunks_bound(int Hout, int Wout, int N);

struct SkinnyArgs {
  const void* X = nullptr;
  const void* W = nullptr;
  void* Y = nullptr;
  int M = 0, N = 0, K = 0, ldx = 0, ldw = 0, ldy = 0;
  int flags = 0;
  float eps = 1e-6f;
  int* bump = nullptr;
  unsigned long long* prof = nullptr;
  const int* pos = nullptr;
  int prof_ld = 0;
  bool x3 = false;
  bool w_shared = false;
  int lds_kb = 0;
  int kind = -1;
  long long* dbg = nullptr;
  const void* next_W = nullptr;
  long next_tile_bytes = 0;
  int next_tiles = 0;
};
#define IVG_GEMM_PROF_SLOTS 8
int launch_skinny(const SkinnyArgs& a, DType dtype, hipStream_t stream);
struct SkinnyPlan { int gen = 0, mf = 0, fn = 0, waves = 0, klw = 0, ring = 0, lg = 0, nburst = 0, wmax = 0, wr = 0, x3 = 0; };
SkinnyPlan skinny_plan(const SkinnyArgs& a, DType dtype);
bool dgemm3_plan(const SkinnyArgs& a, DType dtype, SkinnyPlan& out);
bool dgemm_plan(const SkinnyArgs& a, DType dtype, SkinnyPlan& out);
int launch_dgemm(const SkinnyArgs& a, DType dtype, hipStream_t stream);
int launch_dgemm3(const SkinnyArgs& a, DType dtype, hipStream_t stream);
int dgemm3_w_rows_per_block(const SkinnyArgs& a, DType dtype);
int dgemm_w_rows_per_block(const SkinnyArgs& a, DType dtype);

}
```

ivideogpt_amd/csrc/llama_ops.hip:

```cpp
#include <algorithm>
#include <cstdio>
#include <cstdlib>

#include "ops.h"
#include <atomic>
#include "switches.h"

namespace ivg {

template <typename T>
__global__ __launch_bounds__(256) void embed_kernel(const int64_t* __restrict__ ids, long id_stride, const T* __restrict__ E,
                                                    T* __restrict__ x, long x_bstride, int L, int H, int V) {
  constexpr int VEC = Traits<T>::VEC;
  const int row = blockIdx.x;
  const int b = row / L, l = row - b * L;
  long id = ids[(long)b * id_stride + l];
  id = id < 0 ? 0 : (id >= V ? V - 1 : id);
  const T* src = E + id * H;
  T* dst = x + (long)b * x_bstride + (long)l * H;
  for (int c = threadIdx.x * VEC; c < H; c += 256 * VEC) *(Chunk16*)(dst + c) = *(const Chunk16*)(src + c);
}

int launch_embed(const int64_t* ids, long id_stride, const void* E, void* x, DType dt, int B, int L, int H, int V, hipStream_t st,
                 long x_bstride) {
// ... 104 lines not shown
      T* vd = vc + ((long)bh * Lmax + pos) * HD + c * VEC;
      *(Chunk16*)vd = vlo; *(Chunk16*)(vd + HALF) = vhi;
#pragma unroll
      for (int r = 0; r < DW; ++r) { dst[c * DW + r] = vlo[r]; dst[HALF * (int)sizeof(T) / 4 + c * DW + r] = vhi[r]; }
    } else {
#pragma unroll
      for (int r = 0; r < DW; ++r) { dst[c * DW + r] = 0u; dst[HALF * (int)sizeof(T) / 4 + c * DW + r] = 0u; }
    }
  }
  __syncthreads();
  if (vt) {
    constexpr int PER = ROWS / 4;
    const int d = tid >> 2, lc = tid & 3;
    const T* svT = (const T*)sv;
    T* out = vt + ((long)bh * HD + d) * ldvt + l0 + lc * PER;
    T vals[PER];
#pragma unroll
    for (int j = 0; j < PER; ++j) vals[j] = svT[(long)(lc * PER + j) * (PITCH * 4 / (int)sizeof(T)) + d];
#pragma unroll
    for (int j = 0; j < PER; j += VEC) {
      Chunk16 o;
      if constexpr (sizeof(T) == 2) { bf16x8 t8; for (int r = 0; r < 8; ++r) t8[r] = vals[j + r]; o = __builtin_bit_cast(Chunk16, t8); }
      else { f32x4 t4; for (int r = 0; r < 4; ++r) t4[r] = vals[j + r]; o = __builtin_bit_cast(Chunk16, t4); }
      *(Chunk16*)(out + j) = o;
    }
  }
}

int launch_rope_kv(void* qkv, void* kc, void* vc, void* vt, int ldvt, const float* cosT, const float* sinT, int B, int L,
                   int heads, int hd, int Lmax, const StepState* state, int pos0, DType dt, hipStream_t st) {
  const long total = (long)B * L * heads * (hd / 2);
  if (total <= 0) return 0;
  const int rows = dt == BF16 ? 64 : 32;
  if (hd == 64 && !state && (!vt || (ldvt % rows == 0 && ldvt >= cdiv(L, rows) * rows)) && ((uintptr_t)qkv & 15) == 0) {
    dim3 g2((unsigned)(vt ? ldvt / rows : cdiv(L, rows)), (unsigned)(B * heads));
    if (dt == BF16)
      hipLaunchKernelGGL(rope_kv64_kernel<bf16_t>, g2, dim3(256), 0, st, (bf16_t*)qkv, (bf16_t*)kc, (bf16_t*)vc, (bf16_t*)vt, ldvt, cosT, sinT,
                         L, heads, Lmax, pos0);
    else
      hipLaunchKernelGGL(rope_kv64_kernel<float>, g2, dim3(256), 0, st, (float*)qkv, (float*)kc, (float*)vc, (float*)vt, ldvt, cosT, sinT, L,
                         heads, Lmax, pos0);
    return (int)hipGetLastError();
  }
  if (vt && !state && ldvt > L) {
    const size_t es = dt == BF16 ? 2 : 4;
    const hipError_t rc = hipMemset2DAsync((char*)vt + (size_t)L * es, (size_t)ldvt * es, 0, (size_t)(ldvt - L) * es, (size_t)B * heads * hd, st);
    if (rc != hipSuccess) return (int)rc;
  }
  dim3 g(cdiv(total, 256));
  if (dt == BF16)
    hipLaunchKernelGGL(rope_kv_kernel<bf16_t>, g, dim3(256), 0, st, (bf16_t*)qkv, (bf16_t*)kc, (bf16_t*)vc, (bf16_t*)vt, ldvt, cosT,
                       sinT, B, L, heads, hd, Lmax, state, pos0);
  else
    hipLaunchKernelGGL(rope_kv_kernel<float>, g, dim3(256), 0, st, (float*)qkv, (float*)kc, (float*)vc, (float*)vt, ldvt, cosT, sinT,
                       B, L, heads, hd, Lmax, state, pos0);
  return (int)hipGetLastError();
}

template <int KT>
struct VtTile {
  static constexpr bool SWZ = KT == 32;
  static constexpr int PITCH = SWZ ? KT : KT + 16;
  static __device__ __forceinline__ int quad_off(int row, int quad) {
    if constexpr (SWZ) quad ^= (row >> 1) & 3;
    return row * PITCH + (quad << 3);
  }
  static __device__ __forceinline__ void store(bf16_t* sV, int row, int cc, Chunk16 c) {
    typedef uint32_t U2 __attribute__((ext_vector_type(2)));
    const int qa = (cc >> 2) * 4 + 2 * (cc & 1), e = ((cc >> 1) & 1) * 4;
    bf16_t* a = sV + quad_off(row, qa) + e;
    bf16_t* b = sV + quad_off(row, qa + 1) + e;
    const U2 lo = {c.x, c.y}, hi = {c.z, c.w};
    const bool odd = !SWZ && (row & 1);
    bf16_t* p0 = odd ? b : a;
    bf16_t* p1 = odd ? a : b;
    *(U2*)p0 = odd ? hi : lo;
    *(U2*)p1 = odd ? lo : hi;
  }
  static __device__ __forceinline__ bf16x8 frag(const bf16_t* sV, int row, int quad) { return *(const bf16x8*)(sV + quad_off(row, quad)); }
};

__global__ __launch_bounds__(256) void flash_prefill_kernel(const bf16_t* __restrict__ qkv, const bf16_t* __restrict__ kc,
                                                            const bf16_t* __restrict__ vt, bf16_t* __restrict__ out, int L, int Lp,
                                                            int heads, int Lmax, float scale) {
  constexpr int HD = 64;
  const int tid = threadIdx.x, wave = tid >> 6, lane = tid & 63, lr = lane & 15, lg = lane >> 4;
  const int qt = gridDim.x - 1 - blockIdx.x;
  const int bh = blockIdx.y, b = bh / heads, h = bh - b * heads;
  const int H = heads * HD;
  const int q = qt * 64 + wave * 16 + lr;
  const int qc = q < L ? q : L - 1;
  const bf16_t* qrow = qkv + ((long)b * L + qc) * 3 * H + h * HD;
  const bf16x8 qf0 = *(const bf16x8*)(qrow + lg * 8), qf1 = *(const bf16x8*)(qrow + 32 + lg * 8);
  const bf16_t* kb = kc + (long)bh * Lmax * HD;
  const bf16_t* vb = vt + (long)bh * HD * Lp;
  f32x4 o[4];
#pragma unroll
  for (int d = 0; d < 4; ++d) o[d] = f32x4{0.f, 0.f, 0.f, 0.f};
  float m = -INFINITY, lsum = 0.f;
  using VT = VtTile<64>;
  constexpr int PITCHK = HD + 16;
  __shared__ __attribute__((aligned(16))) bf16_t sK[64 * PITCHK];
  __shared__ __attribute__((aligned(16))) bf16_t sV[64 * VT::PITCH];
  const int srow0 = tid >> 3, scol = (tid & 7) * 8;
  Chunk16 pk[2], pv[2];
  auto fetch = [&](int kt) {
    const int k0 = kt * 64;
#pragma unroll
    for (int i = 0; i < 2; ++i) {
      const int row = srow0 + i * 32;
      const int kr = k0 + row;
      pk[i] = *(const Chunk16*)(kb + (long)(kr < Lmax ? kr : Lmax - 1) * HD + scol);
      pv[i] = *(const Chunk16*)(vb + (long)row * Lp + k0 + scol);
    }
  };
  fetch(0);
  for (int kt = 0; kt <= qt; ++kt) {
    const int k0 = kt * 64;
    __syncthreads();
#pragma unroll
    for (int i = 0; i < 2; ++i) {
      *(Chunk16*)(sK + (srow0 + i * 32) * PITCHK + scol) = pk[i];
      VT::store(sV, srow0 + i * 32, tid & 7, pv[i]);
    }
    __syncthreads();
    if (kt < qt) fetch(kt + 1);
    bf16x8 kf[4][2];
#pragma unroll
    for (int sub = 0; sub < 4; ++sub) {
      const bf16_t* krow = sK + (sub * 16 + lr) * PITCHK;
      kf[sub][0] = *(const bf16x8*)(krow + lg * 8);
      kf[sub][1] = *(const bf16x8*)(krow + 32 + lg * 8);
    }
    bf16x8 vf[4][2];
#pragma unroll
    for (int d = 0; d < 4; ++d)
#pragma unroll
      for (int pr = 0; pr < 2; ++pr) vf[d][pr] = VT::frag(sV, d * 16 + lr, pr * 4 + lg);
    f32x4 sc[4];
    float mt = -INFINITY;
#pragma unroll
    for (int sub = 0; sub < 4; ++sub) {
      sc[sub] = f32x4{0.f, 0.f, 0.f, 0.f};
      sc[sub] = __builtin_amdgcn_mfma_f32_16x16x32_bf16(kf[sub][0], qf0, sc[sub], 0, 0, 0);
      sc[sub] = __builtin_amdgcn_mfma_f32_16x16x32_bf16(kf[sub][1], qf1, sc[sub], 0, 0, 0);
#pragma unroll
      for (int r = 0; r < 4; ++r) {
        const int key = k0 + sub * 16 + lg * 4 + r;
        sc[sub][r] = key <= q ? sc[sub][r] * scale : -INFINITY;
        mt = fmaxf(mt, sc[sub][r]);
      }
    }
    mt = fmaxf(mt, __shfl_xor(mt, 16, 64));
    mt = fmaxf(mt, __shfl_xor(mt, 32, 64));
    const float mn = fmaxf(m, mt);
    const float alpha = expf(m - mn);
    m = mn;
    float ps = 0.f;
    bf16x8 pf[2];
#pragma unroll
    for (int sub = 0; sub < 4; ++sub)
#pragma unroll
      for (int r = 0; r < 4; ++r) {
        const float pv = expf(sc[sub][r] - mn);
        ps += pv;
        pf[sub >> 1][(sub & 1) * 4 + r] = (bf16_t)pv;
      }
    lsum = lsum * alpha + ps;
#pragma unroll
    for (int d = 0; d < 4; ++d) {
#pragma unroll
      for (int r = 0; r < 4; ++r) o[d][r] *= alpha;
#pragma unroll
      for (int pr = 0; pr < 2; ++pr) o[d] = __builtin_amdgcn_mfma_f32_16x16x32_bf16(vf[d][pr], pf[pr], o[d], 0, 0, 0);
    }
  }
  lsum += __shfl_xor(lsum, 16, 64);
  lsum += __shfl_xor(lsum, 32, 64);
  if (q < L) {
    const float inv = 1.0f / lsum;
    bf16_t* orow = out + ((long)b * L + q) * H + h * HD + lg * 4;
#pragma unroll
    for (int d = 0; d < 4; ++d)
      *(bf16x4*)(orow + d * 16) = bf16x4{(bf16_t)(o[d][0] * inv), (bf16_t)(o[d][1] * inv), (bf16_t)(o[d][2] * inv), (bf16_t)(o[d][3] * inv)};
  }
}

int launch_flash_prefill(const void* qkv, const void* kc, const void* vt, void* out, int B, int L, int Lp, int heads, int hd, int Lmax,
                         DType dt, hipStream_t st) {
  if (dt != BF16 || hd != 64 || L <= 0 || Lp % 64 != 0 || Lp < L) return -1;
  dim3 grid((unsigned)cdiv(L, 64), (unsigned)(B * heads));
  hipLaunchKernelGGL(flash_prefill_kernel, grid, dim3(256), 0, st, (const bf16_t*)qkv, (const bf16_t*)kc, (const bf16_t*)vt, (bf16_t*)out, L,
                     Lp, heads, Lmax, 1.0f / sqrtf((float)hd));
  return (int)hipGetLastError();
}

template <int HD, int KT, bool PRE = true>
__global__ __launch_bounds__(256) void xattn_kernel(const bf16_t* __restrict__ q, const bf16_t* __restrict__ Kp, const bf16_t* __restrict__ VpT,
                                                    bf16_t* __restrict__ out, int P, int kv, int C, int F, int nh, float scale) {
  constexpr int KQ = HD / 32;
  constexpr int DO = HD / 16;
  constexpr int SUB = KT / 16;
  constexpr int NPF = KT / 32;
  const int tid = threadIdx.x, wave = tid >> 6, lane = tid & 63, lr = lane & 15, lg = lane >> 4;
  const int qt = blockIdx.x;
  const int mh = blockIdx.y, m = mh / nh, h = mh - m * nh, b = m / F;
  const int qi = qt * 64 + wave * 16 + lr;
  const bf16_t* qrow = q + ((long)m * P + qi) * C + h * HD;
  bf16x8 qf[KQ];
#pragma unroll
  for (int k = 0; k < KQ; ++k) qf[k] = *(const bf16x8*)(qrow + k * 32 + lg * 8);
  const bf16_t* kb = Kp + (long)b * kv * C + h * HD;
  const bf16_t* vb = VpT + ((long)b * C + h * HD) * kv;
  f32x4 o[DO];
#pragma unroll
  for (int d = 0; d < DO; ++d) o[d] = f32x4{0.f, 0.f, 0.f, 0.f};
  float mx = -INFINITY, lsum = 0.f;
  constexpr int PK = HD + 16;
  using VT = VtTile<KT>;
  __shared__ __attribute__((aligned(16))) bf16_t sK[KT * PK];
  __shared__ __attribute__((aligned(16))) bf16_t sV[HD * VT::PITCH];
  constexpr int KC = KT * HD / 8 / 256;
  constexpr int VC = HD * KT / 8 / 256;
  constexpr int VCH = KT / 8;
  static_assert(KC >= 1 && VC >= 1, "tile too small for 256 threads");
  Chunk16 pk[KC], pvv[VC];
  auto fetch = [&](int kt) {
    const int k0 = kt * KT;
#pragma unroll
    for (int i = 0; i < KC; ++i) {
      const int c = i * 256 + tid, row = c / (HD / 8), col = (c % (HD / 8)) * 8;
      pk[i] = *(const Chunk16*)(kb + (long)(k0 + row) * C + col);
    }
#pragma unroll
    for (int i = 0; i < VC; ++i) {
      const int c = i * 256 + tid, row = c / VCH, col = (c % VCH) * 8;
      pvv[i] = *(const Chunk16*)(vb + (long)row * kv + k0 + col);
    }
  };
  const int ntiles = kv / KT;
  if constexpr (PRE) fetch(0);
  for (int kt = 0; kt < ntiles; ++kt) {
    __syncthreads();
    if constexpr (!PRE) fetch(kt);
#pragma unroll
    for (int i = 0; i < KC; ++i) { const int c = i * 256 + tid; *(Chunk16*)(sK + (c / (HD / 8)) * PK + (c % (HD / 8)) * 8) = pk[i]; }
#pragma unroll
    for (int i = 0; i < VC; ++i) { const int c = i * 256 + tid; VT::store(sV, c / VCH, c % VCH, pvv[i]); }
    __syncthreads();
    if constexpr (PRE) { if (kt + 1 < ntiles) fetch(kt + 1); }
    f32x4 sc[SUB];
    float mt = -INFINITY;
#pragma unroll
    for (int sub = 0; sub < SUB; ++sub) {
      sc[sub] = f32x4{0.f, 0.f, 0.f, 0.f};
      const bf16_t* krow = sK + (sub * 16 + lr) * PK + lg * 8;
#pragma unroll
      for (int k = 0; k < KQ; ++k) sc[sub] = __builtin_amdgcn_mfma_f32_16x16x32_bf16(*(const bf16x8*)(krow + k * 32), qf[k], sc[sub], 0, 0, 0);
#pragma unroll
      for (int r = 0; r < 4; ++r) { sc[sub][r] *= scale; mt = fmaxf(mt, sc[sub][r]); }
    }
    mt = fmaxf(mt, __shfl_xor(mt, 16, 64));
    mt = fmaxf(mt, __shfl_xor(mt, 32, 64));
    const float mn = fmaxf(mx, mt);
    const float alpha = expf(mx - mn);
    mx = mn;
    float ps = 0.f;
    bf16x8 pf[NPF];
#pragma unroll
    for (int sub = 0; sub < SUB; ++sub)
#pragma unroll
      for (int r = 0; r < 4; ++r) {
        const float pe = expf(sc[sub][r] - mn);
        ps += pe;
        pf[sub >> 1][(sub & 1) * 4 + r] = (bf16_t)pe;
      }
// ... 1157 lines not shown
    float val = to_f32(src[c]);
    if (act) val += to_f32(act[c]);
    dst[c] = from_f32<T>(val);
  }
}

template <typename T, int KPT, bool NUCLEUS>
static void launch_sample_t(const SampleArgs& a, int B, size_t smem, hipStream_t st) {
  static DynLdsOnce once;
  (void)ensure_dyn_lds(once, (const void*)sample_embed_kernel<T, KPT, NUCLEUS>, 96 * 1024);
  hipLaunchKernelGGL((sample_embed_kernel<T, KPT, NUCLEUS>), dim3(B), dim3(256), smem, st, a);
}

template <bool NUCLEUS>
static void launch_sample_dt(const SampleArgs& a, int B, DType dt, size_t smem, hipStream_t st) {
  const bool small = a.V <= 256 * 36;
  if (dt == BF16) { if (small) launch_sample_t<bf16_t, 36, NUCLEUS>(a, B, smem, st); else launch_sample_t<bf16_t, 72, NUCLEUS>(a, B, smem, st); }
  else { if (small) launch_sample_t<float, 36, NUCLEUS>(a, B, smem, st); else launch_sample_t<float, 72, NUCLEUS>(a, B, smem, st); }
}

int launch_sample_embed(const SampleArgs& a, int B, DType dt, hipStream_t st) {
  const size_t smem = (size_t)std::max(a.V, SAMPLE_CAP) * sizeof(float);
  if (a.V > 256 * 72 || smem > 96 * 1024) return (int)hipErrorInvalidValue;
  if (a.top_p < 1.0f)
    launch_sample_dt<true>(a, B, dt, std::max(smem, (size_t)SAMPLE_CAP * sizeof(double)), st);
  else
    launch_sample_dt<false>(a, B, dt, smem, st);
  return (int)hipGetLastError();
}

__global__ void state_set_kernel(StepState* s, int pos, int j) { s->pos = pos; s->j = j; }

int launch_state_set(StepState* state, int pos, int j, hipStream_t st) {
  hipLaunchKernelGGL(state_set_kernel, dim3(1), dim3(1), 0, st, state, pos, j);
  return (int)hipGetLastError();
}

__global__ void expand_prompt_rows_kernel(const int64_t* __restrict__ prompts, long pstride, int64_t* __restrict__ ids, long ids_ld, int L,
                                          int G, int b0) {
  const int r = blockIdx.y;
  const int64_t* src = prompts + (long)((b0 + r) / G) * pstride;
  for (int c = blockIdx.x * blockDim.x + threadIdx.x; c < L; c += gridDim.x * blockDim.x) ids[(long)r * ids_ld + c] = src[c];
}

int launch_expand_prompt_rows(const int64_t* prompts, long pstride, int64_t* ids, long ids_ld, int rows, int L, int G, int b0, hipStream_t st) {
  if (rows <= 0 || L <= 0) return 0;
  hipLaunchKernelGGL(expand_prompt_rows_kernel, dim3((unsigned)((L + 255) / 256), (unsigned)rows), dim3(256), 0, st, prompts, pstride, ids, ids_ld, L, G, b0);
  return (int)hipGetLastError();
}

template <typename T>
__global__ __launch_bounds__(256) void action_embed_kernel(const float* __restrict__ act, const float* __restrict__ W,
                                                           const float* __restrict__ bias, T* __restrict__ out, int A, int H) {
  const int row = blockIdx.x;
  for (int c = threadIdx.x; c < H; c += 256) {
    float s = 0.f;
    for (int k = 0; k < A; ++k) s = fmaf(act[(long)row * A + k], W[(long)c * A + k], s);
    out[(long)row * H + c] = from_f32<T>(s + bias[c]);
  }
}

int launch_action_embed(const float* act, const float* W, const float* bias, void* out, DType dt, int BT, int A, int H,
                        hipStream_t st) {
  if (BT <= 0) return 0;
  if (dt == BF16) hipLaunchKernelGGL(action_embed_kernel<bf16_t>, dim3(BT), dim3(256), 0, st, act, W, bias, (bf16_t*)out, A, H);
  else hipLaunchKernelGGL(action_embed_kernel<float>, dim3(BT), dim3(256), 0, st, act, W, bias, (float*)out, A, H);
  return (int)hipGetLastError();
}

template <typename T>
__global__ __launch_bounds__(256) void add_rows_kernel(T* __restrict__ x, long xs, const T* __restrict__ add, long as, int H) {
  const int b = blockIdx.x;
  for (int c = threadIdx.x; c < H; c += 256) x[b * xs + c] = from_f32<T>(to_f32(x[b * xs + c]) + to_f32(add[b * as + c]));
}

int launch_add_rows(void* x, long x_stride, const void* add, long add_stride, int B, int H, DType dt, hipStream_t st) {
  if (B <= 0) return 0;
  if (dt == BF16) hipLaunchKernelGGL(add_rows_kernel<bf16_t>, dim3(B), dim3(256), 0, st, (bf16_t*)x, x_stride, (const bf16_t*)add, add_stride, H);
  else hipLaunchKernelGGL(add_rows_kernel<float>, dim3(B), dim3(256), 0, st, (float*)x, x_stride, (const float*)add, add_stride, H);
  return (int)hipGetLastError();
}

template <typename T>
__global__ __launch_bounds__(64) void rowdot_kernel(const T* __restrict__ h, const float* __restrict__ w,
                                                    const float* __restrict__ bias, float* __restrict__ out, int H, float eps) {
  const int b = blockIdx.x;
  float s = 0.f, ss = 0.f;
  for (int c = threadIdx.x; c < H; c += 64) { const float v = to_f32(h[(long)b * H + c]); s = fmaf(v, w[c], s); ss = fmaf(v, v, ss); }
  s = wave_sum(s);
  ss = wave_sum(ss);
  if (threadIdx.x == 0) out[b] = (eps >= 0.f ? s * rsqrtf(ss / (float)H + eps) : s) + bias[0];
}

int launch_rowdot(const void* h, const float* w, const float* bias, float* out, int B, int H, float eps, DType dt, hipStream_t st) {
  if (B <= 0) return 0;
  if (dt == BF16) hipLaunchKernelGGL(rowdot_kernel<bf16_t>, dim3(B), dim3(64), 0, st, (const bf16_t*)h, w, bias, out, H, eps);
  else hipLaunchKernelGGL(rowdot_kernel<float>, dim3(B), dim3(64), 0, st, (const float*)h, w, bias, out, H, eps);
  return (int)hipGetLastError();
}

template <typename T>
__global__ __launch_bounds__(256) void final_hidden_kernel(const T* __restrict__ x, const float* __restrict__ w, T* __restrict__ out,
                                                           int H, float eps) {
  __shared__ float red[4];
  const int b = blockIdx.x, tid = threadIdx.x;
  float ss = 0.f;
  for (int c = tid; c < H; c += 256) { const float v = to_f32(x[(long)b * H + c]); ss = fmaf(v, v, ss); }
  ss = wave_sum(ss);
  if ((tid & 63) == 0) red[tid >> 6] = ss;
  __syncthreads();
  const float rs = rsqrtf(((red[0] + red[1]) + (red[2] + red[3])) / (float)H + eps);
  for (int c = tid; c < H; c += 256) {
    const T n = from_f32<T>(to_f32(x[(long)b * H + c]) * rs);
    out[(long)b * H + c] = from_f32<T>(to_f32(from_f32<T>(w[c])) * to_f32(n));
  }
}

int launch_final_hidden(const void* x, const float* w, void* out, int B, int H, float eps, DType dt, hipStream_t st) {
  if (B <= 0) return 0;
  if (dt == BF16) hipLaunchKernelGGL(final_hidden_kernel<bf16_t>, dim3(B), dim3(256), 0, st, (const bf16_t*)x, w, (bf16_t*)out, H, eps);
  else hipLaunchKernelGGL(final_hidden_kernel<float>, dim3(B), dim3(256), 0, st, (const float*)x, w, (float*)out, H, eps);
  return (int)hipGetLastError();
}

__global__ __launch_bounds__(256) void ce_rows_kernel(const float* __restrict__ logits, const int64_t* __restrict__ labels, long row0,
                                                      int L, int V, float* __restrict__ nll) {
  __shared__ float red[8];
  const long r = row0 + blockIdx.x;
  const int l = (int)(r % L), tid = threadIdx.x, lane = tid & 63, wv = tid >> 6;
  const long tgt = l + 1 < L ? labels[r + 1] : -100;
  if (tgt < 0 || tgt >= V) { if (tid == 0) nll[r] = 0.f; return; }
  const float* row = logits + (long)blockIdx.x * V;
  float mx = -INFINITY;
  for (int i = tid; i < V; i += 256) mx = fmaxf(mx, row[i]);
  mx = wave_max(mx);
  if (lane == 0) red[wv] = mx;
  __syncthreads();
  mx = fmaxf(fmaxf(red[0], red[1]), fmaxf(red[2], red[3]));
  float sum = 0.f;
  for (int i = tid; i < V; i += 256) sum += expf(row[i] - mx);
  sum = wave_sum(sum);
  if (lane == 0) red[4 + wv] = sum;
  __syncthreads();
  if (tid == 0) nll[r] = logf((red[4] + red[5]) + (red[6] + red[7])) + mx - row[tgt];
}

int launch_ce_rows(const float* logits, const int64_t* labels, long row0, int rows, int L, int V, float* nll, hipStream_t st) {
  if (rows <= 0) return 0;
  hipLaunchKernelGGL(ce_rows_kernel, dim3((unsigned)rows), dim3(256), 0, st, logits, labels, row0, L, V, nll);
  return (int)hipGetLastError();
}

__global__ __launch_bounds__(256) void ce_reduce_kernel(const float* __restrict__ nll, const int64_t* __restrict__ labels, int L, int V,
                                                        float* __restrict__ out) {
  __shared__ float rs[4], rc[4];
  const int b = blockIdx.x, tid = threadIdx.x;
  float s = 0.f, c = 0.f;
  for (int l = tid; l + 1 < L; l += 256) {
    const long t = labels[(long)b * L + l + 1];
    if (t >= 0 && t < V) { s += nll[(long)b * L + l]; c += 1.f; }
  }
  s = wave_sum(s); c = wave_sum(c);
  if ((tid & 63) == 0) { rs[tid >> 6] = s; rc[tid >> 6] = c; }
  __syncthreads();
  if (tid == 0) { out[2 * b] = (rs[0] + rs[1]) + (rs[2] + rs[3]); out[2 * b + 1] = (rc[0] + rc[1]) + (rc[2] + rc[3]); }
}
// ... 62 lines not shown
```

ivideogpt_amd/csrc/ops.h:

```cpp
#pragma once
#include "common.h"
#include "igemm.h"

namespace ivg {

int gn_num_chunks(int P);
int launch_groupnorm(const void* X, void* Y, void* part_ws, const float* gamma, const float* beta, const float* pos,
                     int N, int P, int C, int groups, float eps, int silu, DType dt, hipStream_t st);
int launch_groupnorm_partial(const void* X, void* part_ws, int N, int P, int C, int groups, DType dt, hipStream_t st);
int launch_gn_coef(const void* part, int nchunks, const float* gamma, const float* beta, int N, int P, int C, int groups, float eps, void* coef,
                   hipStream_t st);
int launch_groupnorm_apply(const void* X, void* Y, const void* part, int nchunks, const float* gamma, const float* beta, const float* pos,
                           int N, int P, int C, int groups, float eps, int silu, DType dt, hipStream_t st);
int launch_add_rmsnorm(void* x, long x_stride, const float* w, void* out, int M, int H, float eps, DType dt, hipStream_t st);
int launch_softmax(const float* S, void* Pm, long rows, int Lq, int Lk, int lds, int ldp, int causal, DType dt, hipStream_t st);

int launch_conv_in(const void* video, DType video_dt, const float* w , const float* bias, void* Y, DType dt,
                   int N, int per, int T_total, int t0, int H, int W, int C0, hipStream_t st);

struct TokMap {
  int tpf, nf;
  long stride;
  int start, fstride;
};
int launch_sqnorm_rows(const float* E, float* out, int rows, int dim, hipStream_t st);
int launch_vq_argmin(const float* z, const float* E, const float* ee, int64_t* out, const TokMap& map, int64_t offset, int R,
                     int n_e, hipStream_t st);
int launch_gather_rows(const int64_t* ids, const TokMap& map, const float* E, void* Y, DType dt, int R, int dim, int64_t sub,
                       int n_e, hipStream_t st);
int launch_unpatchify(const void* q, void* out, DType dt, int M, int np, int C, int p, hipStream_t st);
int launch_finish_tokens(int64_t* ids, long stride, int64_t* labels, int B, int L, int ctx, int64_t scf, int64_t sdf, hipStream_t st);

struct StepState {
  int pos;
  int j;
};
int launch_embed(const int64_t* ids, long id_stride, const void* E, void* x, DType dt, int B, int L, int H, int V, hipStream_t st,
                 long x_bstride = 0);
int launch_rope_kv(void* qkv, void* kc, void* vc, void* vt, int ldvt, const float* cosT, const float* sinT, int B, int L,
                   int heads, int hd, int Lmax, const StepState* state, int pos0, DType dt, hipStream_t st);
int launch_flash_prefill(const void* qkv, const void* kc, const void* vt, void* out, int B, int L, int Lp, int heads, int hd, int Lmax,
                         DType dt, hipStream_t st);
int launch_xattn(const void* q, const void* Kp, const void* VpT, void* out, int M, int F, int P, int kv, int C, int nh, DType dt, hipStream_t st);
bool xattn_covers(int P, int kv, int C, int nh, DType dt);
#define IVG_ATTN_PROF_SLOTS 32
bool decode_attn_covers(int hd, DType dt);
int launch_decode_attn(const void* qkv, void* kc, void* vc, void* out, const float* cosT, const float* sinT, int B, int heads, int hd,
                       int Lmax, const StepState* state, unsigned long long* prof, DType dt, hipStream_t st, int sh_P = 0, int sh_G = 1,
                       int sh_row0 = 0);
int launch_decode_attn24(const void* qkv, void* kc, void* vc, void* out, const float* cosT, const float* sinT, int B, int heads, int Lmax,
                         const StepState* state, unsigned long long* prof, hipStream_t st, int sh_P = 0, int sh_G = 1, int sh_row0 = 0);
long long decode_attn24_launches();
int launch_kv24_pack(const void* k32, const void* v32, void* kc, void* vc, int BH, int L, int Lmax, hipStream_t st);
int launch_decode_attn8(const void* qkv, void* kc, void* vc, void* out, const float* cosT, const float* sinT, int B, int heads, int Lmax,
                        const StepState* state, unsigned long long* prof, float k_scale, float v_scale, hipStream_t st, int sh_P = 0, int sh_G = 1,
                        int sh_row0 = 0, const float* k_scales = nullptr, const float* v_scales = nullptr);
long long decode_attn8_launches();
int launch_kv8_pack(const void* k16, const void* v16, void* kc, void* vc, int BH, int L, int Lmax, float k_scale, float v_scale, hipStream_t st,
                    int heads = 1, const float* k_scales = nullptr, const float* v_scales = nullptr);
int launch_kv_absmax(const void* k16, const void* v16, int B, int heads, int L, int Lmax, unsigned int* amax, hipStream_t st);
bool kv8_scale_ok(float s);
int launch_expand_prompt_rows(const int64_t* prompts, long pstride, int64_t* ids, long ids_ld, int rows, int L, int G, int b0, hipStream_t st);
struct SampleArgs {
  const float* logits; int V;
  const float* uniforms; int n_uni;
  int top_k;
  int64_t* ids_out; long ids_stride; int L0;
  int forced_period; int64_t forced_token;
  const void* E; void* x; int H;
  const void* act; int act_T; int ctx;
  int slot0;
  StepState* state;
  float temperature;
  float top_p = 1.0f;
};
int launch_sample_embed(const SampleArgs& a, int B, DType dt, hipStream_t st);
int launch_state_set(StepState* state, int pos, int j, hipStream_t st);
int launch_action_embed(const float* act, const float* W, const float* bias, void* out, DType dt, int BT, int A, int H,
                        hipStream_t st);
int launch_add_rows(void* x, long x_stride, const void* add, long add_stride, int B, int H, DType dt, hipStream_t st);
int launch_rowdot(const void* h, const float* w, const float* bias, float* out, int B, int H, float eps, DType dt, hipStream_t st);
int launch_final_hidden(const void* x, const float* w, void* out, int B, int H, float eps, DType dt, hipStream_t st);
int launch_ce_rows(const float* logits, const int64_t* labels, long row0, int rows, int L, int V, float* nll, hipStream_t st);
int launch_ce_reduce(const float* nll, const int64_t* labels, int B, int L, int V, float* out, hipStream_t st);
int launch_action_recon(const void* hidden, const float* W, const float* bias, const float* act, int B, int L, int H, int A, int act_T,
                        int ctx, int prelude, float* out, DType dt, hipStream_t st);
int launch_compare_rows(const void* a, long a_stride_bytes, const void* b, long b_stride_bytes, int rows, long row_bytes, int* flag,
                        hipStream_t st);

int launch_ingest(const unsigned char* src, int T, int H, int W, int crop, void* dst, DType dst_dt, int R, hipStream_t st);

size_t frame_metrics_ws_bytes(int n_samples, int T, int H, int W);
int launch_frame_metrics(const void* gt, DType gt_dt, int B, int T_gt, int gt_t0, const float* pred, int n_samples, int T_pr, int pr_t0, int T,
                         int H, int W, float* rows, void* ws, hipStream_t st);

bool lpips_shape_ok(int H, int W);
size_t lpips_ws_bytes(int max_images, int H, int W);
long lpips_ws_images(size_t ws_bytes, int H, int W);
long long lpips_trunk_images();
int launch_maxpool2(const float* X, float* Y, int N, int H, int W, int C, hipStream_t st);
int launch_lpips_input_layer(const void* images, DType dt, const float* w, const float* bias, float* Y, int n, int H, int W, hipStream_t st);
size_t lpips_head_part_bytes(int n1, int P);
int launch_lpips_head(const float* f0, const float* f1, const float* lin, int n0, int n1, int P, int C, float* out, long group_stride, int accumulate,
                      double* part, hipStream_t st);
int launch_lpips_features(const float* const* cw, const float* const* cb, const void* images, DType dt, int n, int H, int W, float* const* taps_out,
                          void* ws, size_t ws_bytes, hipStream_t st);
int launch_lpips_rows(const float* const* cw, const float* const* cb, const float* const* lin, const void* gt, DType gt_dt, int B, int T_gt, int gt_t0,
                      const float* pred, int n_samples, int T_pr, int pr_t0, int T, int H, int W, float* frames, float* rows, void* ws, size_t ws_bytes,
                      hipStream_t st);

}
```

ivideogpt_amd/csrc/switches.cpp:

```cpp
#include "switches.h"

#include <algorithm>
#include <atomic>
#include <cstdio>
#include <cstdlib>
#include <mutex>

namespace ivg {

static int env_int(const char* name, int dflt) {
  const char* v = getenv(name);
  return (v && v[0]) ? atoi(v) : dflt;
}

static Switches read_env() {
  Switches s;
  const bool dev = env_int("IVG_DEV", 0) == 1;
  auto dv = [&](const char* name, int dflt) { return dev ? env_int(name, dflt) : dflt; };
  s.conv3x3 = dv("IVG_CONV3X3", 1) != 0;
  s.subpixel = dv("IVG_SUBPIXEL", 1) != 0;
  s.gemm256 = dv("IVG_GEMM256", 1) != 0;
  s.gemm256x3 = dv("IVG_GEMM256X3", 1) != 0;
  s.kv24 = dv("IVG_KV24", 1) != 0;
  s.dg3 = dv("IVG_DG3", 1) != 0;
  s.flash_prefill = dv("IVG_FLASH_PREFILL", 1) != 0;
  s.flash_xatt = dv("IVG_FLASH_XATT", 1) != 0;
  s.gn_fuse = dv("IVG_GN_FUSE", 1) != 0;
  s.gn_apply_fuse = dv("IVG_GN_APPLY_FUSE", 1) != 0;
  s.x3 = dv("IVG_X3", 1) != 0;
  s.dg3_warm = dv("IVG_DG3_WARM", 1) != 0;
  s.warm_gate_up = dv("IVG_WARM_GATE_UP", 0) != 0;
  s.conv_cap = dv("IVG_CONV_CAP", 0) == 1;
  s.decode_w_shared = dv("IVG_DECODE_W_SHARED", 1) != 0;
  s.inflight_warm = dv("IVG_INFLIGHT_WARM", 0) != 0;
  s.dg2_mf_cap = dv("IVG_DG2_MF_CAP", 0);
  if (s.dg2_mf_cap != 1 && s.dg2_mf_cap != 2) s.dg2_mf_cap = 0;
  s.inflight_gemm256 = dv("IVG_INFLIGHT_GEMM256", 1) != 0;
  if (const char* v = dev ? getenv("IVG_INFLIGHT_KB") : nullptr) {
    int k[5] = {0, 0, 0, 0, 0};
    if (sscanf(v, "%d,%d,%d,%d,%d", &k[0], &k[1], &k[2], &k[3], &k[4]) == 5)
      for (int i = 0; i < 5; ++i) s.inflight_kb[i] = (k[i] >= 16 && k[i] <= 160) ? k[i] : 0;
  }
  s.graph = env_int("IVG_GRAPH", 0) == 1;
  s.decode_lds_kb = env_int("IVG_DECODE_LDS_KB", 160);
  if (s.decode_lds_kb < 16 || s.decode_lds_kb > 160) s.decode_lds_kb = 160;
  return s;
}

bool Switches::operator==(const Switches& o) const {
  return conv3x3 == o.conv3x3 && subpixel == o.subpixel && gemm256 == o.gemm256 && dg3 == o.dg3 && flash_prefill == o.flash_prefill &&
         flash_xatt == o.flash_xatt && gn_fuse == o.gn_fuse && gn_apply_fuse == o.gn_apply_fuse && x3 == o.x3 && gemm256x3 == o.gemm256x3 && kv24 == o.kv24 && graph == o.graph &&
         dg3_warm == o.dg3_warm && warm_gate_up == o.warm_gate_up && conv_cap == o.conv_cap && decode_lds_kb == o.decode_lds_kb && decode_w_shared == o.decode_w_shared &&
         inflight_warm == o.inflight_warm && dg2_mf_cap == o.dg2_mf_cap && inflight_gemm256 == o.inflight_gemm256 &&
         std::equal(inflight_kb, inflight_kb + 5, o.inflight_kb);
}

static std::atomic<const Switches*> g_cur{nullptr};
static std::atomic<unsigned> g_gen{0};
static std::mutex g_mu;

void reload_switches() {
  std::lock_guard<std::mutex> lk(g_mu);
  const Switches now = read_env();
  const Switches* cur = g_cur.load(std::memory_order_acquire);
  if (cur && *cur == now) return;
  g_cur.store(new Switches(now), std::memory_order_release);
  g_gen.fetch_add(1, std::memory_order_release);
}

const Switches& sw() {
  const Switches* p = g_cur.load(std::memory_order_acquire);
  if (!p) { reload_switches(); p = g_cur.load(std::memory_order_acquire); }
  return *p;
}

unsigned switches_generation() { return g_gen.load(std::memory_order_acquire); }

}
```

ivideogpt_amd/csrc/switches.h:

```cpp
#pragma once

namespace ivg {

struct Switches {
  int conv3x3 = 1, subpixel = 1, gemm256 = 1, dg3 = 1, flash_prefill = 1, flash_xatt = 1, gn_fuse = 1, gn_apply_fuse = 1, x3 = 1, gemm256x3 = 1, kv24 = 1;
  int graph = 0, dg3_warm = 1, warm_gate_up = 0, conv_cap = 0, decode_lds_kb = 160, decode_w_shared = 1, inflight_warm = 0, dg2_mf_cap = 0, inflight_gemm256 = 1;
  int inflight_kb[5] = {0, 0, 0, 0, 0};
  bool operator==(const Switches& o) const;
};

const Switches& sw();
void reload_switches();
unsigned switches_generation();

}
```

ivideogpt_amd/csrc/tokenizer.cpp:

```cpp
#include "engine_impl.h"
#include "switches.h"

namespace ivg {

#define CK(x) do { int _e = (x); if (_e != 0) return R.e->fail(IVG_ERR_HIP, std::string(#x) + " failed: hip error " + std::to_string(_e)); } while (0)

static size_t esz(DType d) { return d == BF16 ? 2 : 4; }

static bool gn_fuse_enabled() { return sw().gn_fuse != 0; }

size_t Run::gn_stats_bytes(int N, int H, int W, int C) const {
  return (size_t)N * conv3x3_gn_chunks_bound(H, W, C) * e->cfg.norm_num_groups * sizeof(double) * 2;
}

int Run::conv(DType dt, const void* X, int N, int H, int W, const ConvW& c, void* Y, int stride, int ups, const void* Rres, int flags,
              int out_f32, GnStats* out_stats, const void* in_coef) {
  Run& R = *this;
  if (out_stats) out_stats->chunks = 0;
  const int k = c.k;
  int Ho, Wo, pad;
  if (ups) { Ho = 2 * H; Wo = 2 * W; pad = 1; }
  else if (stride == 2) { Ho = H / 2; Wo = W / 2; pad = 0; }
  else if (stride == k && k > 1) { Ho = H / k; Wo = W / k; pad = 0; }
  else { Ho = H; Wo = W; pad = (k - 1) / 2; }
  IgemmArgs a;
  a.X = X; a.W = c.w; a.Y = Y; a.R = Rres; a.bias = c.b;
  a.Nimg = N; a.Hin = H; a.Win = W; a.Cin = c.cin; a.ldx = c.cin; a.Hout = Ho; a.Wout = Wo;
  a.KH = k; a.KW = k; a.stride = stride; a.pad = pad; a.ups = ups;
  a.N = c.cout; a.ldw = k * k * c.cin;
  a.c_img = (long)Ho * Wo * c.cout; a.c_pix = c.cout; a.c_ch = 1;
  a.flags = flags | (c.b ? IG_BIAS_N : 0) | (Rres ? IG_RESIDUAL : 0) | (out_f32 ? IG_OUT_F32 : 0);
  if (planning) return 0;
  if (out_stats && out_stats->part && gn_fuse_enabled()) { a.gn_part = out_stats->part; a.gn_groups = e->cfg.norm_num_groups; }
  a.gn_in_coef = in_coef;
  if (dt == F32 && x3 && sw().x3) { a.x3 = true; a.W_x3 = c.w3; }
  if (ups) { a.W_sub = c.wsub; a.W_sub_x3 = a.W_x3 ? c.wsub3 : nullptr; }
  const double flops = 2.0 * N * Ho * Wo * (double)c.cout * k * k * c.cin;
  const double bytes = (double)esz(dt) * ((double)N * H * W * c.cin + (double)c.cout * k * k * c.cin) + (double)(out_f32 ? 4 : esz(dt)) * N * Ho * Wo * c.cout;
  if (k == 3 && stride == 1) {
    prof_begin(dt, flops, bytes, 2);
    const int rc = launch_conv3x3(a, dt, st);
    if (rc == 0) { prof_end(dt, 2); if (out_stats) out_stats->chunks = a.gn_chunks; return 0; }
    prof_cancel(dt, 2);
    if (rc > 0) CK(rc);
  }
  if (in_coef) return -100;
  prof_begin(dt, flops, bytes);
  int rc = -1;
  if (k == 1 && stride == 1 && !ups) rc = launch_gemm256(a, dt, st);
  if (rc == -1) rc = launch_igemm(a, dt, st);
  CK(rc);
  prof_end(dt);
  return 0;
}

int Run::gemm(DType dt, const IgemmArgs& a0, double flops, double bytes) {
  Run& R = *this;
  if (planning) return 0;
  IgemmArgs a = a0;
  a.x3 = dt == F32 && x3 && sw().x3;
  prof_begin(dt, flops, bytes);
  int rc = -1;
  if (!(e->in_flight() && !sw().inflight_gemm256)) rc = launch_gemm256(a, dt, st);
  if (rc == -1) rc = launch_igemm(a, dt, st);
  CK(rc);
  prof_end(dt);
  return 0;
}

int Run::linear(DType dt, const void* X, long rows, const ConvW& c, void* Y, const void* Rres, int flags, int out_f32) {
  IgemmArgs a;
  a.X = X; a.W = c.w; a.Y = Y; a.R = Rres; a.bias = c.b;
  a.Nimg = 1; a.Hin = 1; a.Win = (int)rows; a.Cin = c.cin; a.ldx = c.cin; a.Hout = 1; a.Wout = (int)rows;
  a.N = c.cout; a.ldw = c.cin;
  a.c_img = 0; a.c_pix = c.cout; a.c_ch = 1;
  a.flags = flags | (c.b ? IG_BIAS_N : 0) | (Rres ? IG_RESIDUAL : 0) | (out_f32 ? IG_OUT_F32 : 0);
  return gemm(dt, a, 2.0 * rows * c.cin * (double)c.cout,
              (double)esz(dt) * ((double)rows * c.cin + (double)c.cout * c.cin) + (double)(out_f32 ? 4 : esz(dt)) * rows * c.cout);
}

int Run::gnorm(DType dt, const void* X, void* Y, int N, int P, int C, const NormW& n, float eps, int silu, const float* pos,
               const GnStats* stats) {
  Run& R = *this;
  const int groups = e->cfg.norm_num_groups;
  if (stats && stats->part && stats->chunks > 0 && !planning) {
    CK(launch_groupnorm_apply(X, Y, stats->part, stats->chunks, n.g, n.b, pos, N, P, C, groups, eps, silu, dt, st));
    return 0;
  }
  const size_t m = e->ws.mark();
  void* part = e->ws.alloc((size_t)N * gn_num_chunks(P) * groups * sizeof(double) * 2);
  int rc = 0;
  if (!planning) rc = launch_groupnorm(X, Y, part, n.g, n.b, pos, N, P, C, groups, eps, silu, dt, st);
  e->ws.reset(m);
  CK(rc);
  return 0;
}

static bool gn_apply_fuse_enabled() { return sw().gn_apply_fuse != 0; }

int Run::norm_conv(DType dt, const void* x, int N, int H, int W, const NormW& n, float eps, const GnStats* x_stats, const ConvW& c, void* Y,
                   const void* Rres, void* scratch, GnStats* out_stats) {
  Run& R = *this;
  const int groups = e->cfg.norm_num_groups, P = H * W, C = c.cin;
  const size_t m = e->ws.mark();
  void* part = e->ws.alloc((size_t)N * gn_num_chunks(P) * groups * sizeof(double) * 2);
  void* coef = e->ws.alloc((size_t)N * C * sizeof(float) * 2);
  int rc = 0;
  if (!planning) {
    const bool fuse = gn_apply_fuse_enabled() && c.k == 3;
    const void* st_part = x_stats && x_stats->chunks > 0 ? x_stats->part : nullptr;
    int chunks = st_part ? x_stats->chunks : 0;
    if (!st_part) {
      CK(launch_groupnorm_partial(x, part, N, P, C, groups, dt, st));
      st_part = part; chunks = gn_num_chunks(P);
    }
    rc = -100;
    if (fuse) {
      CK(launch_gn_coef(st_part, chunks, n.g, n.b, N, P, C, groups, eps, coef, st));
      rc = conv(dt, x, N, H, W, c, Y, 1, 0, Rres, 0, 0, out_stats, coef);
    }
    if (rc == -100) {
      CK(launch_groupnorm_apply(x, scratch, st_part, chunks, n.g, n.b, nullptr, N, P, C, groups, eps, 1, dt, st));
      rc = conv(dt, scratch, N, H, W, c, Y, 1, 0, Rres, 0, 0, out_stats);
    }
  } else if (out_stats) {
    out_stats->chunks = 0;
  }
  e->ws.reset(m);
  return rc;
}

int Run::resnet(DType dt, const void* x, int N, int H, int W, const ResnetW& r, void* out, const GnStats* x_stats, GnStats* out_stats) {
  Run& R = *this;
  const size_t m = e->ws.mark();
  const size_t px = (size_t)N * H * W;
  void* t = e->ws.alloc(px * std::max(r.cin, r.cout) * esz(dt));
  void* h = e->ws.alloc(px * r.cout * esz(dt));
  GnStats hs;
  hs.part = e->ws.alloc(gn_stats_bytes(N, H, W, r.cout));
  IVG_TRY(norm_conv(dt, x, N, H, W, r.n1, 1e-6f, x_stats, r.c1, h, nullptr, t, &hs));
  const void* res = x;
  if (r.has_sc) {
    IVG_TRY(conv(dt, x, N, H, W, r.sc, out, 1, 0, nullptr, 0, 0));
    res = out;
  }
  IVG_TRY(norm_conv(dt, h, N, H, W, r.n2, 1e-6f, &hs, r.c2, out, res, t, out_stats));
  e->ws.reset(m);
  return 0;
}

int Run::self_attention(DType dt, const void* x, int N, int P, int C, const AttnW& a, void* out) {
  Run& R = *this;
  const size_t m = e->ws.mark();
  const size_t tok = (size_t)N * P;
  void* t = e->ws.alloc(tok * C * esz(dt));
  void* q = e->ws.alloc(tok * C * esz(dt));
  void* k = e->ws.alloc(tok * C * esz(dt));
  void* vT = e->ws.alloc(tok * C * esz(dt));
  void* o = e->ws.alloc(tok * C * esz(dt));
// ... 450 lines not shown
```

ivideogpt_amd/csrc/transformer.cpp:

```cpp
#include <cstring>
#include "engine_impl.h"
#include "switches.h"

namespace ivg {

#define CK(x) do { int _e = (x); if (_e != 0) return e->fail(IVG_ERR_HIP, std::string(#x) + " failed: hip error " + std::to_string(_e)); } while (0)

static size_t esz(DType d) { return d == BF16 ? 2 : 4; }
static size_t rup(size_t v, size_t a) { return (v + a - 1) / a * a; }

struct GenBuf {
  StepState* state;
  char* x; char* qkv; char* attn; char* act; float* logits;
  int64_t* ids; float* uni; char* act_emb; int Bc, ids_ld;
  float* last_act;
  int* flag;
  int sh_P = 0, sh_G = 1, sh_row0 = 0;
};

static size_t gen_layout(const ivg_engine* e, GenBuf& g, char* base) {
  const ivg_config& c = e->cfg;
  const DType dt = e->llm_dt;
  const int Bc = e->kvc.chunk, H = c.hidden_size, I = c.intermediate_size, V = c.vocab_size;
  g.Bc = Bc;
  g.ids_ld = e->Lmax;
  size_t off = 0;
  auto take = [&](size_t bytes) { char* p = base ? base + off : nullptr; off = rup(off + bytes, 256); return p; };
  g.state = (StepState*)take(256);
  g.x = take((size_t)Bc * H * esz(dt));
  g.qkv = take((size_t)Bc * 3 * H * esz(dt));
  g.attn = take((size_t)Bc * H * esz(dt));
  g.act = take((size_t)Bc * I * esz(dt));
  g.logits = (float*)take((size_t)Bc * V * 4);
  g.ids = (int64_t*)take((size_t)Bc * g.ids_ld * 8);
  g.uni = (float*)take((size_t)Bc * g.ids_ld * 4);
  g.act_emb = take((size_t)Bc * std::max(1, c.max_frames) * H * esz(dt));
  g.last_act = (float*)take((size_t)Bc * std::max(1, c.max_frames) * std::max(1, c.action_dim) * 4);
  g.flag = (int*)take(256);
  return off;
}

size_t gen_buffer_bytes(const ivg_engine* e) {
  GenBuf g;
  return gen_layout(e, g, nullptr);
}

static bool flash_prefill_covers(DType dt, int hd) {
  return sw().flash_prefill && dt == BF16 && hd == 64;
}

int Run::prefill(const PrefillReq& q) {
  const ivg_config& c = e->cfg;
  const KvCache& kvc = e->kvc;
  const int B = q.B, L = q.L;
  const DType dt = e->llm_dt;
  x3 = e->llm_x3;
  const int H = c.hidden_size, I = c.intermediate_size, V = c.vocab_size, heads = e->heads, hd = e->hd, Lmax = e->Lmax;
  const long M = (long)B * L;
  const int Lp = (int)rup(L, 64);
  const size_t m = e->ws.mark();
  char* x = (char*)e->ws.alloc((size_t)M * H * esz(dt));
  char* xn = (char*)e->ws.alloc((size_t)M * H * esz(dt));
  char* qkv = (char*)e->ws.alloc((size_t)M * 3 * H * esz(dt));
  char* attn = (char*)e->ws.alloc((size_t)M * H * esz(dt));
  char* act = (char*)e->ws.alloc((size_t)M * I * esz(dt));
  const bool flash = flash_prefill_covers(dt, hd);
  float* S = flash ? nullptr : (float*)e->ws.alloc((size_t)B * heads * L * Lp * 4);
  char* stage_k = kvc.staged() ? (char*)e->ws.alloc(kvc.stage_bytes(B)) : nullptr;
  char* stage_v = kvc.staged() ? (char*)e->ws.alloc(kvc.stage_bytes(B)) : nullptr;
  char* Pm = flash ? nullptr : (char*)e->ws.alloc((size_t)B * heads * L * Lp * esz(dt));
  if (!planning) {
    e->kvc.forget_kept();
    if (q.embeds) CK((int)hipMemcpyAsync(x, q.embeds, (size_t)M * H * esz(dt), hipMemcpyDeviceToDevice, st));
    else CK(launch_embed(q.ids, q.ids_stride, e->embed, x, dt, B, L, H, V, st));
    if (q.act_emb) {
      for (int i = 0;; ++i) {
        const int pos = 257 * q.ctx - 1 + 17 * i;
        if (pos >= L || i + q.ctx - 1 >= q.act_T) break;
        CK(launch_add_rows(x + (size_t)pos * H * esz(dt), (long)L * H, (const char*)q.act_emb + (size_t)(i + q.ctx - 1) * H * esz(dt),
                           (long)q.act_T * H, B, H, dt, st));
        if (!q.all_slots) break;
      }
    }
  }
  for (int l = 0; l < c.num_layers; ++l) {
    const LayerW& w = e->layers[l];
    if (!planning) CK(launch_add_rmsnorm(x, H, e->ones, xn, (int)M, H, c.rms_norm_eps, dt, st));
    ConvW wq; wq.w = w.wqkv; wq.cin = H; wq.cout = 3 * H;
    IVG_TRY(linear(dt, xn, M, wq, qkv, nullptr, 0, 0));
    char* kl = stage_k ? stage_k : kvc.ptr(l, 0);
    char* vl = stage_v ? stage_v : kvc.ptr(l, 1);
    if (!planning) {
      CK(launch_rope_kv(qkv, kl, vl, e->vt, Lp, e->rope_cos, e->rope_sin, B, L, heads, hd, Lmax, nullptr, 0, dt, st));
      if (kv_amax) CK(launch_kv_absmax(kl, vl, B, heads, L, Lmax, kv_amax + (size_t)l * 2 * heads, st));
      CK(kvc.store_staged(l, stage_k, stage_v, B, L, st));
    }
    if (flash) {
      if (!planning) CK(launch_flash_prefill(qkv, kl, e->vt, attn, B, L, Lp, heads, hd, Lmax, dt, st));
    } else {
    {
      IgemmArgs g;
      g.X = qkv; g.W = kl; g.Y = S;
      g.Nimg = 1; g.Hin = 1; g.Win = L; g.Cin = hd; g.ldx = 3 * H; g.Hout = 1; g.Wout = L;
      g.N = L; g.ldw = hd; g.c_pix = Lp; g.c_ch = 1; g.flags = IG_OUT_F32; g.alpha = 1.0f / sqrtf((float)hd);
      g.nb0 = B; g.nb1 = heads;
      g.sa[0] = (long)L * 3 * H; g.sa[1] = hd;
      g.sw[0] = (long)heads * Lmax * hd; g.sw[1] = (long)Lmax * hd;
      g.sy[0] = (long)heads * L * Lp; g.sy[1] = (long)L * Lp;
      IVG_TRY(gemm(dt, g, 2.0 * B * heads * (double)L * L * hd, (double)esz(dt) * 2.0 * M * H + 4.0 * B * heads * L * Lp));
    }
    if (!planning) CK(launch_softmax(S, Pm, (long)B * heads * L, L, L, Lp, Lp, 1, dt, st));
    {
      IgemmArgs g;
      g.X = Pm; g.W = e->vt; g.Y = attn;
      g.Nimg = 1; g.Hin = 1; g.Win = L; g.Cin = Lp; g.ldx = Lp; g.Hout = 1; g.Wout = L;
      g.N = hd; g.ldw = Lp; g.c_pix = H; g.c_ch = 1;
      g.nb0 = B; g.nb1 = heads;
      g.sa[0] = (long)heads * L * Lp; g.sa[1] = (long)L * Lp;
      g.sw[0] = (long)heads * hd * Lp; g.sw[1] = (long)hd * Lp;
      g.sy[0] = (long)L * H; g.sy[1] = hd;
      IVG_TRY(gemm(dt, g, 2.0 * B * heads * (double)L * Lp * hd, (double)esz(dt) * ((double)B * heads * L * Lp + 2.0 * M * H)));
    }
    }
    ConvW wo; wo.w = w.wo; wo.cin = H; wo.cout = H;
    IVG_TRY(linear(dt, attn, M, wo, x, x, 0, 0));
    if (!planning) CK(launch_add_rmsnorm(x, H, e->ones, xn, (int)M, H, c.rms_norm_eps, dt, st));
    {
      IgemmArgs g;
      g.X = xn; g.W = w.wgu; g.Y = act;
      g.Nimg = 1; g.Hin = 1; g.Win = (int)M; g.Cin = H; g.ldx = H; g.Hout = 1; g.Wout = (int)M;
      g.N = 2 * I; g.ldw = H; g.c_pix = I; g.c_ch = 1; g.flags = IG_GLU;
      IVG_TRY(gemm(dt, g, 2.0 * M * (double)H * 2 * I, (double)esz(dt) * ((double)M * H + 2.0 * I * H + (double)M * I)));
    }
    ConvW wd; wd.w = w.wdown; wd.cin = I; wd.cout = H;
    IVG_TRY(linear(dt, act, M, wd, x, x, 0, 0));
  }
  if (q.hidden_all && !planning) {
    if (!e->final_norm) return e->fail(IVG_ERR_MISSING, "hidden states requested but 'llm.norm' is not in the weight table");
    CK(launch_final_hidden(x, e->final_norm, q.hidden_all, (int)M, H, c.rms_norm_eps, dt, st));
  }
  if (q.logits_all) {
    if (!planning) CK(launch_add_rmsnorm(x, H, e->ones, xn, (int)M, H, c.rms_norm_eps, dt, st));
    ConvW wl; wl.w = e->lm_head; wl.cin = H; wl.cout = V;
    IVG_TRY(linear(dt, xn, M, wl, q.logits_all, nullptr, 0, 1));
  }
  if (q.token_nll) {
    const long Rc = std::min<long>(M, 4096);
    float* chunk = (float*)e->ws.alloc((size_t)Rc * V * 4);
    if (!planning && !q.logits_all) CK(launch_add_rmsnorm(x, H, e->ones, xn, (int)M, H, c.rms_norm_eps, dt, st));
    ConvW wl; wl.w = e->lm_head; wl.cin = H; wl.cout = V;
    for (long r0 = 0; r0 < M; r0 += Rc) {
      const long rows = std::min(Rc, M - r0);
      IVG_TRY(linear(dt, xn + (size_t)r0 * H * esz(dt), rows, wl, chunk, nullptr, 0, 1));
      if (!planning) CK(launch_ce_rows(chunk, q.labels, r0, (int)rows, L, V, q.token_nll, st));
    }
  }
  if (q.logits_last && !planning) {
    CK((int)hipMemcpy2DAsync(q.hidden_last, (size_t)H * esz(dt), x + (size_t)(L - 1) * H * esz(dt), (size_t)L * H * esz(dt),
                             (size_t)H * esz(dt), B, hipMemcpyDeviceToDevice, st));
    SkinnyArgs s;
    s.X = q.hidden_last; s.W = e->lm_head; s.Y = q.logits_last; s.M = B; s.N = V; s.K = H; s.ldx = H; s.ldw = H; s.ldy = V;
    s.flags = IG_OUT_F32 | SK_NORM; s.eps = c.rms_norm_eps; s.lds_kb = e->decode_lds_kb;
    s.w_shared = e->in_flight() && sw().decode_w_shared;
    CK(launch_skinny(s, dt, st));
  }
  e->ws.reset(m);
  return 0;
}

static int step_body(ivg_engine* e, hipStream_t st, const GenBuf& g, int B, const SampleArgs& sa, bool forward, bool skip_sample = false) {
  const ivg_config& c = e->cfg;
  const DType dt = e->llm_dt;
  const int H = c.hidden_size, I = c.intermediate_size, V = c.vocab_size;
  const size_t es = esz(dt);
  StepState* state = g.state;
  char* x = g.x; char* qkv = g.qkv; char* attn = g.attn; char* act = g.act; float* logits = g.logits;
  if (!skip_sample) CK(launch_sample_embed(sa, B, dt, st));
  if (!forward) return 0;
  const size_t gp_ld = (size_t)IVG_GEMM_PROF_SLOTS * 2 * e->Lmax;
  auto gprof = [&](SkinnyArgs& a, int idx) {
    if (!e->gemm_prof_on || !e->gemm_prof) return;
    a.prof = e->gemm_prof + (size_t)idx * gp_ld; a.pos = (const int*)state; a.prof_ld = e->Lmax;
  };
  const bool in_flight = e->in_flight();
  const bool w_shared = in_flight && sw().decode_w_shared;
  const bool warm = !in_flight || sw().inflight_warm;
  auto link_next = [&](SkinnyArgs& cur, const SkinnyArgs& nxt) {
    if (!warm) return;
    if ((nxt.flags & IG_GLU) && !sw().warm_gate_up) return;
    int rows = dgemm3_w_rows_per_block(nxt, dt);
    if (rows <= 0) rows = dgemm_w_rows_per_block(nxt, dt);
    if (rows <= 0 || nxt.ldw != nxt.K) return;
    cur.next_W = nxt.W; cur.next_tile_bytes = (long)rows * nxt.K * (long)es; cur.next_tiles = nxt.N / rows;
  };
  auto layer_args = [&](int l, SkinnyArgs* g) {
    const LayerW& w = e->layers[l];
    for (int k = 0; k < 4; ++k) {
      g[k].x3 = e->llm_x3 && sw().x3; g[k].lds_kb = e->decode_lds_kb; g[k].w_shared = w_shared; g[k].kind = k;
      if (in_flight && sw().inflight_kb[k] > 0) g[k].lds_kb = sw().inflight_kb[k];
    }
    SkinnyArgs& s = g[0];
    s.X = x; s.W = w.wqkv; s.Y = qkv; s.M = B; s.N = 3 * H; s.K = H; s.ldx = H; s.ldw = H; s.ldy = 3 * H;
    s.flags = SK_NORM; s.eps = c.rms_norm_eps;
    SkinnyArgs& o = g[1];
    o.X = attn; o.W = w.wo; o.Y = x; o.M = B; o.N = H; o.K = H; o.ldx = H; o.ldw = H; o.ldy = H; o.flags = IG_RESIDUAL;
    SkinnyArgs& u = g[2];
    u.X = x; u.W = w.wgu; u.Y = act; u.M = B; u.N = 2 * I; u.K = H; u.ldx = H; u.ldw = H; u.ldy = I;
    u.flags = IG_GLU | SK_NORM; u.eps = c.rms_norm_eps;
    SkinnyArgs& d = g[3];
    d.X = act; d.W = w.wdown; d.Y = x; d.M = B; d.N = H; d.K = I; d.ldx = I; d.ldw = I; d.ldy = H; d.flags = IG_RESIDUAL;
  };
  SkinnyArgs lm;
  lm.X = x; lm.W = e->lm_head; lm.Y = logits; lm.M = B; lm.N = V; lm.K = H; lm.ldx = H; lm.ldw = H; lm.ldy = V;
  lm.flags = IG_OUT_F32 | SK_NORM; lm.eps = c.rms_norm_eps; lm.lds_kb = e->decode_lds_kb; lm.w_shared = w_shared; lm.kind = 4;
  if (in_flight && sw().inflight_kb[4] > 0) lm.lds_kb = sw().inflight_kb[4];
  lm.bump = (int*)state;
  SkinnyArgs cur[4], nxt[4];
  layer_args(0, cur);
  for (int l = 0; l < c.num_layers; ++l) {
    const bool last = l + 1 == c.num_layers;
    if (!last) layer_args(l + 1, nxt);
    link_next(cur[0], cur[1]); link_next(cur[1], cur[2]); link_next(cur[2], cur[3]); link_next(cur[3], last ? lm : nxt[0]);
    gprof(cur[0], 4 * l + 0);
    CK(launch_skinny(cur[0], dt, st));
    unsigned long long* aprof = e->attn_prof_on ? e->attn_prof + (size_t)l * IVG_ATTN_PROF_SLOTS * 2 * e->Lmax : nullptr;
    CK(e->kvc.decode_attn(l, qkv, attn, e->rope_cos, e->rope_sin, B, state, aprof, st, g.sh_P, g.sh_G, g.sh_row0));
    gprof(cur[1], 4 * l + 1);
    CK(launch_skinny(cur[1], dt, st));
    gprof(cur[2], 4 * l + 2);
    CK(launch_skinny(cur[2], dt, st));
    gprof(cur[3], 4 * l + 3);
    CK(launch_skinny(cur[3], dt, st));
    if (!last) for (int k = 0; k < 4; ++k) cur[k] = nxt[k];
  }
  {
    SkinnyArgs first[4];
    layer_args(0, first);
    link_next(lm, first[0]);
  }
  gprof(lm, 4 * c.num_layers);
  CK(launch_skinny(lm, dt, st));
  return 0;
// ... 206 lines not shown
```

Before: 5579 predicted frames/s.

## Prune last prefill layer to final rows and add tiled conv_in kernel

```diff
diff --git a/include/ivg.h b/include/ivg.h
--- a/include/ivg.h
+++ b/include/ivg.h
@@ -198,6 +198,8 @@
                               int pos, int P, int G, int row0, int dtype, ivg_stream stream);
 int ivg_op_prefill_attn(void* qkv, void* kc, void* vc, void* vt, void* out, const float* cos_t, const float* sin_t, int B, int L, int heads, int hd,
                         int Lmax, int dtype, ivg_stream stream);
+int ivg_op_prefill_logits_last(ivg_engine* e, const int64_t* ids, int64_t ids_stride, int B, int L, const float* actions, int act_T, int ctx,
+                               float* logits_out, ivg_stream stream);
 int ivg_op_kv24_pack(const float* k32, const float* v32, void* kc, void* vc, int BH, int L, int Lmax, ivg_stream stream);
 int ivg_op_decode_attn24(const float* qkv, void* kc, void* vc, float* out, const float* cos_t, const float* sin_t, int B, int heads, int Lmax, int pos,
                          int P, int G, int row0, ivg_stream stream);
diff --git a/ivideogpt_amd/_lib.py b/ivideogpt_amd/_lib.py
--- a/ivideogpt_amd/_lib.py
+++ b/ivideogpt_amd/_lib.py
@@ -136,6 +136,7 @@
     "ivg_op_vq_argmin": (C.c_int, [C.c_void_p] * 4 + [C.c_int, C.c_int, C.c_void_p]),
     "ivg_op_add_rmsnorm": (C.c_int, [C.c_void_p, C.c_void_p, C.c_void_p, C.c_int, C.c_int, C.c_float, C.c_int, C.c_void_p]),
     "ivg_op_conv_in": (C.c_int, [C.c_void_p, C.c_int, C.c_void_p, C.c_void_p, C.c_void_p] + [C.c_int] * 8 + [C.c_void_p]),
+    "ivg_op_prefill_logits_last": (C.c_int, [C.c_void_p, C.c_void_p, C.c_int64, C.c_int, C.c_int, C.c_void_p, C.c_int, C.c_int, C.c_void_p, C.c_void_p]),
     "ivg_op_sample": (C.c_int, [C.c_void_p, C.c_int, C.c_int, C.c_int, C.c_float, C.c_void_p, C.c_void_p, C.c_void_p]),
     "ivg_op_sample_top_p": (C.c_int, [C.c_void_p, C.c_int, C.c_int, C.c_int, C.c_float, C.c_float, C.c_void_p, C.c_void_p, C.c_void_p]),
     "ivg_debug_counter": (C.c_int64, [C.c_char_p]),
diff --git a/ivideogpt_amd/csrc/api.cpp b/ivideogpt_amd/csrc/api.cpp
--- a/ivideogpt_amd/csrc/api.cpp
+++ b/ivideogpt_amd/csrc/api.cpp
@@ -691,6 +691,21 @@
   if (actions && (e->cfg.action_dim <= 0 || !e->act_w)) return e->fail(IVG_ERR_INVALID, "logits: actions given but the model is action-free");
   return plan_then_run(e, (hipStream_t)stream, [&](Run& r) {
     PrefillReq q; q.ids = ids; q.ids_stride = L; q.B = B; q.L = L; q.act_T = act_T; q.ctx = ctx; q.all_slots = true; q.logits_all = logits_out;
+    IVG_TRY(embed_actions(r, actions, B * act_T, &q.act_emb));
+    return r.prefill(q);
+  });
+}
+
+int ivg_op_prefill_logits_last(ivg_engine* e, const int64_t* ids, int64_t ids_stride, int B, int L, const float* actions, int act_T, int ctx,
+                               float* logits_out, ivg_stream stream) {
+  if (!e || !ids || !logits_out) return IVG_ERR_INVALID;
+  if (e->cfg.num_layers <= 0) return e->fail(IVG_ERR_INVALID, "prefill_logits_last: engine was created without a transformer");
+  if (B <= 0 || B > e->kvc.chunk || L < 1 || L > e->Lmax || ids_stride < L) return e->fail(IVG_ERR_CAPACITY, "prefill_logits_last: batch or length exceeds capacity");
+  if (actions && (e->cfg.action_dim <= 0 || !e->act_w)) return e->fail(IVG_ERR_INVALID, "prefill_logits_last: actions given but the model is action-free");
+  if (actions && (ctx < 1 || act_T < 1 || act_T > e->cfg.max_frames)) return e->fail(IVG_ERR_INVALID, "prefill_logits_last: bad ctx / act_T");
+  return plan_then_run(e, (hipStream_t)stream, [&](Run& r) {
+    PrefillReq q; q.ids = ids; q.ids_stride = ids_stride; q.B = B; q.L = L; q.act_T = act_T; q.ctx = ctx; q.all_slots = true; q.logits_last = logits_out;
+    q.hidden_last = e->ws.alloc((size_t)B * e->cfg.hidden_size * dtype_size(e->llm_dt));
     IVG_TRY(embed_actions(r, actions, B * act_T, &q.act_emb));
     return r.prefill(q);
   });
@@ -1079,6 +1094,10 @@
   if (name && !strcmp(name, "decode_gemm_gen3")) return decode_gemm_launches(3);
   if (name && !strcmp(name, "decode_gemm_gen2")) return decode_gemm_launches(2);
   if (name && !strcmp(name, "lpips_trunk_images")) return lpips_trunk_images();
+  if (name && !strcmp(name, "conv_in_tiled")) return conv_in_tiled_launches();
+  if (name && !strcmp(name, "prefill_last_full")) return prefill_last_layer_count(0);
+  if (name && !strcmp(name, "prefill_last_rows")) return prefill_last_layer_count(1);
+  if (name && !strcmp(name, "prefill_last_stop")) return prefill_last_layer_count(2);
   return -1;
 }
 
diff --git a/ivideogpt_amd/csrc/common.h b/ivideogpt_amd/csrc/common.h
--- a/ivideogpt_amd/csrc/common.h
+++ b/ivideogpt_amd/csrc/common.h
@@ -82,4 +82,14 @@
   return e;
 }
 
+static inline int device_cu_count() {
+  static std::atomic<int> cached[64];
+  int d = 0, n = 0;
+  (void)hipGetDevice(&d);
+  if ((n = cached[d & 63].load(std::memory_order_relaxed)) > 0) return n;
+  if (hipDeviceGetAttribute(&n, hipDeviceAttributeMultiprocessorCount, d) != hipSuccess || n <= 0) return 256;
+  cached[d & 63].store(n, std::memory_order_relaxed);
+  return n;
 }
+
+}
diff --git a/ivideogpt_amd/csrc/conv_small.hip b/ivideogpt_amd/csrc/conv_small.hip
--- a/ivideogpt_amd/csrc/conv_small.hip
+++ b/ivideogpt_amd/csrc/conv_small.hip
@@ -1,4 +1,8 @@
+#include <algorithm>
+#include <atomic>
+
 #include "ops.h"
+#include "switches.h"
 
 namespace ivg {
 
@@ -54,10 +58,113 @@
   }
 }
 
+constexpr int CI_TP = 64;
+constexpr int CI_PRE = (27 * CI_TP + 255) / 256;
+
+template <typename TI, typename TO>
+__global__ __launch_bounds__(256) void conv_in_tiled_kernel(const TI* __restrict__ video, const float* __restrict__ w,
+                                                            const float* __restrict__ bias, TO* __restrict__ Y, int NP ,
+                                                            int per, int T_total, int t0, int H, int W, int C0, int chunks) {
+  extern __shared__ __attribute__((aligned(16))) unsigned char smem[];
+  float* sw = (float*)smem;
+  float* sb = sw + 27 * C0;
+  float* sp = sb + C0;
+  for (int i = threadIdx.x; i < 27 * C0; i += 256) {
+    const int k = i / C0, co = i - k * C0;
+    sw[i] = w[co * 27 + k];
+  }
+  for (int i = threadIdx.x; i < C0; i += 256) sb[i] = bias[i];
+  const int cgn = C0 / 8, HW = H * W;
+  float pre[CI_PRE];
+  auto fetch = [&](int chunk) {
+#pragma unroll
+    for (int u = 0; u < CI_PRE; ++u) {
+      const int i = u * 256 + threadIdx.x;
+      const int tap = i / CI_TP, p = chunk * CI_TP + (i - tap * CI_TP);
+      float x = 0.f;
+      if (tap < 27 && p < NP) {
+        const int n = p / HW, r = p - n * HW, oh = r / W, ow = r - oh * W;
+        const int ci = tap / 9, kh = (tap - ci * 9) / 3, kw = tap - ci * 9 - kh * 3;
+        const int ih = oh + kh - 1, iw = ow + kw - 1;
+        const long fr = (long)(n / per) * T_total + t0 + (n % per);
+        if (ih >= 0 && ih < H && iw >= 0 && iw < W) x = to_f32(video[(fr * 3 + ci) * HW + (long)ih * W + iw]);
+      }
+      pre[u] = x;
+    }
+  };
+  auto stage = [&](float* dst) {
+#pragma unroll
+    for (int u = 0; u < CI_PRE; ++u) {
+      const int i = u * 256 + threadIdx.x;
+      if (i < 27 * CI_TP) dst[i] = pre[u];
+    }
+  };
+  int chunk = blockIdx.x, buf = 0;
+  fetch(chunk);
+  stage(sp);
+  __syncthreads();
+  for (; chunk < chunks; chunk += gridDim.x, buf ^= 1) {
+    const int next = chunk + gridDim.x;
+    if (next < chunks) fetch(next);
+    const float* px = sp + buf * 27 * CI_TP;
+    for (int it = threadIdx.x; it < (CI_TP / 2) * cgn; it += 256) {
+      const int pp = it / cgn, cg = it - pp * cgn;
+      float acc[2][8];
+#pragma unroll
+      for (int j = 0; j < 8; ++j) acc[0][j] = acc[1][j] = sb[cg * 8 + j];
+#pragma unroll
+      for (int k = 0; k < 27; ++k) {
+        const float x0 = px[k * CI_TP + pp], x1 = px[k * CI_TP + CI_TP / 2 + pp];
+        const float* wk = sw + k * C0 + cg * 8;
+#pragma unroll
+        for (int j = 0; j < 8; ++j) {
+          acc[0][j] = fmaf(x0, wk[j], acc[0][j]);
+          acc[1][j] = fmaf(x1, wk[j], acc[1][j]);
+        }
+      }
+#pragma unroll
+      for (int h = 0; h < 2; ++h) {
+        const int p = chunk * CI_TP + h * (CI_TP / 2) + pp;
+        if (p >= NP) continue;
+        TO* o = Y + (long)p * C0 + cg * 8;
+        if constexpr (sizeof(TO) == 2) {
+          bf16x8 v;
+#pragma unroll
+          for (int j = 0; j < 8; ++j) v[j] = (bf16_t)acc[h][j];
+          *(bf16x8*)o = v;
+        } else {
+          *(f32x4*)o = f32x4{acc[h][0], acc[h][1], acc[h][2], acc[h][3]};
+          *(f32x4*)(o + 4) = f32x4{acc[h][4], acc[h][5], acc[h][6], acc[h][7]};
+        }
+      }
+    }
+    if (next < chunks) stage(sp + (buf ^ 1) * 27 * CI_TP);
+    __syncthreads();
+  }
+}
+
+static std::atomic<long long> g_conv_in_tiled_launches{0};
+long long conv_in_tiled_launches() { return g_conv_in_tiled_launches.load(); }
+
 int launch_conv_in(const void* video, DType video_dt, const float* w, const float* bias, void* Y, DType dt, int N, int per,
                    int T_total, int t0, int H, int W, int C0, hipStream_t st) {
   if (C0 % 8 != 0 || N <= 0) return N <= 0 ? 0 : (int)hipErrorInvalidValue;
   const long total = (long)N * H * W * (C0 / 8);
+  const long npix = (long)N * H * W;
+  if (sw().conv_in_tiled && npix + CI_TP <= 0x7fffffffL && C0 <= 256) {
+    const int chunks = cdiv(npix, CI_TP);
+    const int blocks = std::min(chunks, 4 * device_cu_count());
+    const size_t smem = (size_t)(28 * C0 + 2 * 27 * CI_TP) * sizeof(float);
+    dim3 g(blocks), b(256);
+#define IVG_CI(TI, TO) hipLaunchKernelGGL((conv_in_tiled_kernel<TI, TO>), g, b, smem, st, (const TI*)video, w, bias, (TO*)Y, (int)npix, per, T_total, t0, H, W, C0, chunks)
+    if (video_dt == F32 && dt == F32) IVG_CI(float, float);
+    else if (video_dt == F32 && dt == BF16) IVG_CI(float, bf16_t);
+    else if (video_dt == BF16 && dt == F32) IVG_CI(bf16_t, float);
+    else IVG_CI(bf16_t, bf16_t);
+#undef IVG_CI
+    g_conv_in_tiled_launches.fetch_add(1);
+    return (int)hipGetLastError();
+  }
   const int blocks = (int)(total / 256 > 16384 ? 16384 : cdiv(total, 256));
   const size_t smem = (size_t)(28 * C0) * sizeof(float);
   dim3 g(blocks), b(256);
diff --git a/ivideogpt_amd/csrc/engine_impl.h b/ivideogpt_amd/csrc/engine_impl.h
--- a/ivideogpt_amd/csrc/engine_impl.h
+++ b/ivideogpt_amd/csrc/engine_impl.h
@@ -47,7 +47,7 @@
   int norm_conv(DType dt, const void* x, int N, int H, int W, const NormW& n, float eps, const GnStats* x_stats, const ConvW& c, void* Y,
                 const void* Rres, void* scratch, GnStats* out_stats);
   int gemm(DType dt, const IgemmArgs& a, double flops, double bytes);
-  int linear(DType dt, const void* X, long rows, const ConvW& c, void* Y, const void* Rres, int flags, int out_f32);
+  int linear(DType dt, const void* X, long rows, const ConvW& c, void* Y, const void* Rres, int flags, int out_f32, long sel_rows = 0);
   int gnorm(DType dt, const void* X, void* Y, int N, int P, int C, const NormW& n, float eps, int silu, const float* pos,
             const GnStats* stats = nullptr );
   int resnet(DType dt, const void* x, int N, int H, int W, const ResnetW& r, void* out, const GnStats* x_stats = nullptr,
diff --git a/ivideogpt_amd/csrc/gemm256.hip b/ivideogpt_amd/csrc/gemm256.hip
--- a/ivideogpt_amd/csrc/gemm256.hip
+++ b/ivideogpt_amd/csrc/gemm256.hip
@@ -303,7 +303,8 @@
   if (a.c_ch != 1 || (a.c_grp > 1)) return -1;
   if (a.Nimg > 1 && a.c_img != (long)a.Hout * a.Wout * a.c_pix) return -1;
   const bool glu = a.flags & IG_GLU;
-  if (M < 4096 || a.N % 256 != 0 || a.Cin % 32 != 0 || a.Cin < 64 || a.ldw % 4 != 0 || a.c_pix % 4 != 0) return -1;
+  const long Msel = a.sel_rows > 0 ? a.sel_rows : M;
+  if (M <= 0 || Msel < 4096 || a.N % 256 != 0 || a.Cin % 32 != 0 || a.Cin < 64 || a.ldw % 4 != 0 || a.c_pix % 4 != 0) return -1;
   if (((uintptr_t)a.X & 15) || ((uintptr_t)a.W & 15) || ((uintptr_t)a.Y & 15) || ((a.flags & IG_RESIDUAL) && ((uintptr_t)a.R & 15))) return -1;
   if (glu && (a.flags & IG_BIAS_N)) return -1;
   if ((long)a.N * a.ldw * 4 >= (1L << 32)) return -1;
@@ -345,8 +346,9 @@
   if (a.Nimg > 1 && a.c_img != (long)a.Hout * a.Wout * a.c_pix) return -1;
   const bool glu = a.flags & IG_GLU;
   const int BN = a.N % 256 == 0 ? 256 : 128;
-  if (BN == 128 && (glu || M < (1L << 18))) return -1;
-  if (M < 4096 || M > 0x7fffffffL || a.N % 128 != 0 || a.Cin % 32 != 0 || a.Cin < 64 || a.ldw % 8 != 0 || a.c_pix % 8 != 0) return -1;
+  const long Msel = a.sel_rows > 0 ? a.sel_rows : M;
+  if (BN == 128 && (glu || Msel < (1L << 18))) return -1;
+  if (M <= 0 || Msel < 4096 || M > 0x7fffffffL || a.N % 128 != 0 || a.Cin % 32 != 0 || a.Cin < 64 || a.ldw % 8 != 0 || a.c_pix % 8 != 0) return -1;
   if (((uintptr_t)a.X & 15) || ((uintptr_t)a.W & 15) || ((uintptr_t)a.Y & 15) || ((a.flags & IG_RESIDUAL) && ((uintptr_t)a.R & 7))) return -1;
   if (glu && (a.flags & IG_BIAS_N)) return -1;
   if (a.Cin % 64 != 0 || (long)a.N * a.ldw * 2 >= (1L << 31)) return -1;
diff --git a/ivideogpt_amd/csrc/igemm.h b/ivideogpt_amd/csrc/igemm.h
--- a/ivideogpt_amd/csrc/igemm.h
+++ b/ivideogpt_amd/csrc/igemm.h
@@ -38,6 +38,7 @@
   const void* W_sub = nullptr;
   const void* W_sub_x3 = nullptr;
   bool x3 = false;
+  long sel_rows = 0;
   int nb0 = 1, nb1 = 1, nb2 = 1;
   long sa[3] = {0, 0, 0}, sw[3] = {0, 0, 0}, sy[3] = {0, 0, 0};
 };
@@ -51,6 +52,7 @@
   int stage_ok = 0, gn_off = 0, coef_off = 0;
 };
 Conv3Plan conv3x3_plan(const IgemmArgs& a, DType dtype);
+long long prefill_last_layer_count(int kind);
 long long gemm256x3_launches();
 long long conv3x3_subpixel_launches();
 long long decode_gemm_launches(int generation);
diff --git a/ivideogpt_amd/csrc/llama_ops.hip b/ivideogpt_amd/csrc/llama_ops.hip
--- a/ivideogpt_amd/csrc/llama_ops.hip
+++ b/ivideogpt_amd/csrc/llama_ops.hip
@@ -210,10 +210,10 @@
 
 __global__ __launch_bounds__(256) void flash_prefill_kernel(const bf16_t* __restrict__ qkv, const bf16_t* __restrict__ kc,
                                                             const bf16_t* __restrict__ vt, bf16_t* __restrict__ out, int L, int Lp,
-                                                            int heads, int Lmax, float scale) {
+                                                            int heads, int Lmax, float scale, int qt0) {
   constexpr int HD = 64;
   const int tid = threadIdx.x, wave = tid >> 6, lane = tid & 63, lr = lane & 15, lg = lane >> 4;
-  const int qt = gridDim.x - 1 - blockIdx.x;
+  const int qt = qt0 + gridDim.x - 1 - blockIdx.x;
   const int bh = blockIdx.y, b = bh / heads, h = bh - b * heads;
   const int H = heads * HD;
   const int q = qt * 64 + wave * 16 + lr;
@@ -315,11 +315,12 @@
 }
 
 int launch_flash_prefill(const void* qkv, const void* kc, const void* vt, void* out, int B, int L, int Lp, int heads, int hd, int Lmax,
-                         DType dt, hipStream_t st) {
+                         DType dt, hipStream_t st, int first_qt) {
   if (dt != BF16 || hd != 64 || L <= 0 || Lp % 64 != 0 || Lp < L) return -1;
-  dim3 grid((unsigned)cdiv(L, 64), (unsigned)(B * heads));
+  if (first_qt < 0 || first_qt >= cdiv(L, 64)) return (int)hipErrorInvalidValue;
+  dim3 grid((unsigned)(cdiv(L, 64) - first_qt), (unsigned)(B * heads));
   hipLaunchKernelGGL(flash_prefill_kernel, grid, dim3(256), 0, st, (const bf16_t*)qkv, (const bf16_t*)kc, (const bf16_t*)vt, (bf16_t*)out, L,
-                     Lp, heads, Lmax, 1.0f / sqrtf((float)hd));
+                     Lp, heads, Lmax, 1.0f / sqrtf((float)hd), first_qt);
   return (int)hipGetLastError();
 }
 
@@ -1643,6 +1644,21 @@
 }
 
 template <typename T>
+__global__ __launch_bounds__(256) void gather_last_rows_kernel(const T* __restrict__ a, const T* __restrict__ x, T* __restrict__ da,
+                                                               T* __restrict__ dx, int L, int H) {
+  const int b = blockIdx.x;
+  const long src = ((long)b * L + L - 1) * H;
+  for (int c = threadIdx.x; c < H; c += 256) { da[(long)b * H + c] = a[src + c]; dx[(long)b * H + c] = x[src + c]; }
+}
+
+int launch_gather_last_rows(const void* a, const void* x, void* dst_a, void* dst_x, int B, int L, int H, DType dt, hipStream_t st) {
+  if (B <= 0) return 0;
+  if (dt == BF16) hipLaunchKernelGGL(gather_last_rows_kernel<bf16_t>, dim3(B), dim3(256), 0, st, (const bf16_t*)a, (const bf16_t*)x, (bf16_t*)dst_a, (bf16_t*)dst_x, L, H);
+  else hipLaunchKernelGGL(gather_last_rows_kernel<float>, dim3(B), dim3(256), 0, st, (const float*)a, (const float*)x, (float*)dst_a, (float*)dst_x, L, H);
+  return (int)hipGetLastError();
+}
+
+template <typename T>
 __global__ __launch_bounds__(64) void rowdot_kernel(const T* __restrict__ h, const float* __restrict__ w,
                                                     const float* __restrict__ bias, float* __restrict__ out, int H, float eps) {
   const int b = blockIdx.x;
diff --git a/ivideogpt_amd/csrc/ops.h b/ivideogpt_amd/csrc/ops.h
--- a/ivideogpt_amd/csrc/ops.h
+++ b/ivideogpt_amd/csrc/ops.h
@@ -17,6 +17,7 @@
 
 int launch_conv_in(const void* video, DType video_dt, const float* w , const float* bias, void* Y, DType dt,
                    int N, int per, int T_total, int t0, int H, int W, int C0, hipStream_t st);
+long long conv_in_tiled_launches();
 
 struct TokMap {
   int tpf, nf;
@@ -40,7 +41,8 @@
 int launch_rope_kv(void* qkv, void* kc, void* vc, void* vt, int ldvt, const float* cosT, const float* sinT, int B, int L,
                    int heads, int hd, int Lmax, const StepState* state, int pos0, DType dt, hipStream_t st);
 int launch_flash_prefill(const void* qkv, const void* kc, const void* vt, void* out, int B, int L, int Lp, int heads, int hd, int Lmax,
-                         DType dt, hipStream_t st);
+                         DType dt, hipStream_t st, int first_qt = 0);
+int launch_gather_last_rows(const void* a, const void* x, void* dst_a, void* dst_x, int B, int L, int H, DType dt, hipStream_t st);
 int launch_xattn(const void* q, const void* Kp, const void* VpT, void* out, int M, int F, int P, int kv, int C, int nh, DType dt, hipStream_t st);
 bool xattn_covers(int P, int kv, int C, int nh, DType dt);
 #define IVG_ATTN_PROF_SLOTS 32
diff --git a/ivideogpt_amd/csrc/switches.cpp b/ivideogpt_amd/csrc/switches.cpp
--- a/ivideogpt_amd/csrc/switches.cpp
+++ b/ivideogpt_amd/csrc/switches.cpp
@@ -36,6 +36,8 @@
   s.dg2_mf_cap = dv("IVG_DG2_MF_CAP", 0);
   if (s.dg2_mf_cap != 1 && s.dg2_mf_cap != 2) s.dg2_mf_cap = 0;
   s.inflight_gemm256 = dv("IVG_INFLIGHT_GEMM256", 1) != 0;
+  s.prefill_prune = dv("IVG_PREFILL_PRUNE", 1) != 0;
+  s.conv_in_tiled = dv("IVG_CONV_IN_TILED", 1) != 0;
   if (const char* v = dev ? getenv("IVG_INFLIGHT_KB") : nullptr) {
     int k[5] = {0, 0, 0, 0, 0};
     if (sscanf(v, "%d,%d,%d,%d,%d", &k[0], &k[1], &k[2], &k[3], &k[4]) == 5)
@@ -51,7 +53,7 @@
   return conv3x3 == o.conv3x3 && subpixel == o.subpixel && gemm256 == o.gemm256 && dg3 == o.dg3 && flash_prefill == o.flash_prefill &&
          flash_xatt == o.flash_xatt && gn_fuse == o.gn_fuse && gn_apply_fuse == o.gn_apply_fuse && x3 == o.x3 && gemm256x3 == o.gemm256x3 && kv24 == o.kv24 && graph == o.graph &&
          dg3_warm == o.dg3_warm && warm_gate_up == o.warm_gate_up && conv_cap == o.conv_cap && decode_lds_kb == o.decode_lds_kb && decode_w_shared == o.decode_w_shared &&
-         inflight_warm == o.inflight_warm && dg2_mf_cap == o.dg2_mf_cap && inflight_gemm256 == o.inflight_gemm256 &&
+         inflight_warm == o.inflight_warm && dg2_mf_cap == o.dg2_mf_cap && inflight_gemm256 == o.inflight_gemm256 && prefill_prune == o.prefill_prune && conv_in_tiled == o.conv_in_tiled &&
          std::equal(inflight_kb, inflight_kb + 5, o.inflight_kb);
 }
 
diff --git a/ivideogpt_amd/csrc/switches.h b/ivideogpt_amd/csrc/switches.h
--- a/ivideogpt_amd/csrc/switches.h
+++ b/ivideogpt_amd/csrc/switches.h
@@ -5,6 +5,7 @@
 struct Switches {
   int conv3x3 = 1, subpixel = 1, gemm256 = 1, dg3 = 1, flash_prefill = 1, flash_xatt = 1, gn_fuse = 1, gn_apply_fuse = 1, x3 = 1, gemm256x3 = 1, kv24 = 1;
   int graph = 0, dg3_warm = 1, warm_gate_up = 0, conv_cap = 0, decode_lds_kb = 160, decode_w_shared = 1, inflight_warm = 0, dg2_mf_cap = 0, inflight_gemm256 = 1;
+  int conv_in_tiled = 1, prefill_prune = 1;
   int inflight_kb[5] = {0, 0, 0, 0, 0};
   bool operator==(const Switches& o) const;
 };
diff --git a/ivideogpt_amd/csrc/tokenizer.cpp b/ivideogpt_amd/csrc/tokenizer.cpp
--- a/ivideogpt_amd/csrc/tokenizer.cpp
+++ b/ivideogpt_amd/csrc/tokenizer.cpp
@@ -68,13 +68,14 @@
   return 0;
 }
 
-int Run::linear(DType dt, const void* X, long rows, const ConvW& c, void* Y, const void* Rres, int flags, int out_f32) {
+int Run::linear(DType dt, const void* X, long rows, const ConvW& c, void* Y, const void* Rres, int flags, int out_f32, long sel_rows) {
   IgemmArgs a;
   a.X = X; a.W = c.w; a.Y = Y; a.R = Rres; a.bias = c.b;
   a.Nimg = 1; a.Hin = 1; a.Win = (int)rows; a.Cin = c.cin; a.ldx = c.cin; a.Hout = 1; a.Wout = (int)rows;
   a.N = c.cout; a.ldw = c.cin;
   a.c_img = 0; a.c_pix = c.cout; a.c_ch = 1;
   a.flags = flags | (c.b ? IG_BIAS_N : 0) | (Rres ? IG_RESIDUAL : 0) | (out_f32 ? IG_OUT_F32 : 0);
+  a.sel_rows = sel_rows;
   return gemm(dt, a, 2.0 * rows * c.cin * (double)c.cout,
               (double)esz(dt) * ((double)rows * c.cin + (double)c.cout * c.cin) + (double)(out_f32 ? 4 : esz(dt)) * rows * c.cout);
 }
diff --git a/ivideogpt_amd/csrc/transformer.cpp b/ivideogpt_amd/csrc/transformer.cpp
--- a/ivideogpt_amd/csrc/transformer.cpp
+++ b/ivideogpt_amd/csrc/transformer.cpp
@@ -1,3 +1,4 @@
+#include <atomic>
 #include <cstring>
 #include "engine_impl.h"
 #include "switches.h"
@@ -45,6 +46,9 @@
   return gen_layout(e, g, nullptr);
 }
 
+static std::atomic<long long> g_prefill_tail{0}, g_prefill_stop{0}, g_prefill_full{0};
+long long prefill_last_layer_count(int kind) { return (kind == 0 ? g_prefill_full : kind == 1 ? g_prefill_tail : g_prefill_stop).load(); }
+
 static bool flash_prefill_covers(DType dt, int hd) {
   return sw().flash_prefill && dt == BF16 && hd == 64;
 }
@@ -69,6 +73,13 @@
   char* stage_k = kvc.staged() ? (char*)e->ws.alloc(kvc.stage_bytes(B)) : nullptr;
   char* stage_v = kvc.staged() ? (char*)e->ws.alloc(kvc.stage_bytes(B)) : nullptr;
   char* Pm = flash ? nullptr : (char*)e->ws.alloc((size_t)B * heads * L * Lp * esz(dt));
+  const bool no_rows_out = !q.hidden_all && !q.logits_all && !q.token_nll;
+  const bool prune_stop = sw().prefill_prune && no_rows_out && !q.logits_last;
+  const bool prune_tail = sw().prefill_prune && no_rows_out && q.logits_last && flash;
+  char* attn_c = (char*)e->ws.alloc((size_t)B * H * esz(dt));
+  char* x_c = (char*)e->ws.alloc((size_t)B * H * esz(dt));
+  char* xn_c = (char*)e->ws.alloc((size_t)B * H * esz(dt));
+  char* act_c = (char*)e->ws.alloc((size_t)B * I * esz(dt));
   if (!planning) {
     e->kvc.forget_kept();
     if (q.embeds) CK((int)hipMemcpyAsync(x, q.embeds, (size_t)M * H * esz(dt), hipMemcpyDeviceToDevice, st));
@@ -94,6 +105,26 @@
       CK(launch_rope_kv(qkv, kl, vl, e->vt, Lp, e->rope_cos, e->rope_sin, B, L, heads, hd, Lmax, nullptr, 0, dt, st));
       if (kv_amax) CK(launch_kv_absmax(kl, vl, B, heads, L, Lmax, kv_amax + (size_t)l * 2 * heads, st));
       CK(kvc.store_staged(l, stage_k, stage_v, B, L, st));
+    }
+    const bool last = l == c.num_layers - 1;
+    if (last && !planning) (prune_stop ? g_prefill_stop : prune_tail ? g_prefill_tail : g_prefill_full).fetch_add(1);
+    if (last && prune_stop) break;
+    if (last && prune_tail) {
+      if (!planning) {
+        CK(launch_flash_prefill(qkv, kl, e->vt, attn, B, L, Lp, heads, hd, Lmax, dt, st, (L - 1) / 64));
+        CK(launch_gather_last_rows(attn, x, attn_c, x_c, B, L, H, dt, st));
+      }
+      ConvW wo; wo.w = w.wo; wo.cin = H; wo.cout = H;
+      IVG_TRY(linear(dt, attn_c, B, wo, x_c, x_c, 0, 0, M));
+      if (!planning) CK(launch_add_rmsnorm(x_c, H, e->ones, xn_c, B, H, c.rms_norm_eps, dt, st));
+      IgemmArgs g;
+      g.X = xn_c; g.W = w.wgu; g.Y = act_c;
+      g.Nimg = 1; g.Hin = 1; g.Win = B; g.Cin = H; g.ldx = H; g.Hout = 1; g.Wout = B;
+      g.N = 2 * I; g.ldw = H; g.c_pix = I; g.c_ch = 1; g.flags = IG_GLU; g.sel_rows = M;
+      IVG_TRY(gemm(dt, g, 2.0 * B * (double)H * 2 * I, (double)esz(dt) * ((double)B * H + 2.0 * I * H + (double)B * I)));
+      ConvW wd; wd.w = w.wdown; wd.cin = I; wd.cout = H;
+      IVG_TRY(linear(dt, act_c, B, wd, q.hidden_last, x_c, 0, 0, M));
+      break;
     }
     if (flash) {
       if (!planning) CK(launch_flash_prefill(qkv, kl, e->vt, attn, B, L, Lp, heads, hd, Lmax, dt, st));
@@ -156,8 +187,9 @@
     }
   }
   if (q.logits_last && !planning) {
-    CK((int)hipMemcpy2DAsync(q.hidden_last, (size_t)H * esz(dt), x + (size_t)(L - 1) * H * esz(dt), (size_t)L * H * esz(dt),
-                             (size_t)H * esz(dt), B, hipMemcpyDeviceToDevice, st));
+    if (!prune_tail)
+      CK((int)hipMemcpy2DAsync(q.hidden_last, (size_t)H * esz(dt), x + (size_t)(L - 1) * H * esz(dt), (size_t)L * H * esz(dt),
+                               (size_t)H * esz(dt), B, hipMemcpyDeviceToDevice, st));
     SkinnyArgs s;
     s.X = q.hidden_last; s.W = e->lm_head; s.Y = q.logits_last; s.M = B; s.N = V; s.K = H; s.ldx = H; s.ldw = H; s.ldy = V;
     s.flags = IG_OUT_F32 | SK_NORM; s.eps = c.rms_norm_eps; s.lds_kb = e->decode_lds_kb;
```

New measurement: 5609 predicted frames/s (median of 6 runs). No clear change (+0.5%).
